# SAR-Research-Lab/lvt

Hardware: AMD Instinct MI355X
Metric: stereo frames/sec (KITTI-shaped 1241x376), per-frame SE3 vs CPU ref (higher is better)
Workload: dtype u8/f64

## Files before the change

include/lvt_amd_ext.h:

```cpp
#ifndef LVT_AMD_EXT_H__
#define LVT_AMD_EXT_H__

#include "lvt_c.h"
#include <stdint.h>

#ifdef __cplusplus
extern "C" {
#endif

typedef struct lvt_amd_params {
    float fx, fy, cx, cy;
    float baseline;
    int img_width, img_height;
    float k1, k2, p1, p2, k3;
    float near_plane_distance, far_plane_distance;
    float triangulation_ratio_test_threshold;
    float tracking_ratio_test_threshold;
    float descriptor_matching_threshold;
    int min_num_matches_for_tracking;
    int tracking_radius;
    int detection_cell_size;
    int max_keypoints_per_cell;
    int agast_threshold;
    int untracked_threshold;
    int staged_threshold;
    int triangulation_policy;
} lvt_amd_params;

LVT_API void lvt_amd_default_params(lvt_amd_params *p);
LVT_API int lvt_amd_params_from_file(const char *config_file_name, lvt_amd_params *p);
LVT_API lvt_handle lvt_amd_create(const lvt_amd_params *p, int sensor_type);
LVT_API lvt_handle lvt_amd_create_on_device(const lvt_amd_params *p, int sensor_type, int device);
LVT_API int lvt_amd_get_device(lvt_handle h);
LVT_API lvt_handle lvt_amd_create_pooled(const lvt_amd_params *p, int sensor_type, int device );
LVT_API void lvt_amd_reset(lvt_handle h);
LVT_API void lvt_amd_track_rgbd(lvt_handle h, const unsigned char *gray, const float *depth, int n_rows,
                                int n_cols, double R[3][3], double t[3]);
LVT_API void lvt_amd_track_device(lvt_handle h, const void *d_left, const void *d_right, int n_rows,
                                  int n_cols, int pitch_bytes, double R[3][3], double t[3]);
LVT_API void lvt_amd_track_device_async(lvt_handle h, const void *d_left, const void *d_right, int n_rows,
                                        int n_cols, int pitch_bytes);
LVT_API int lvt_amd_track_async(lvt_handle h, const unsigned char *left, const unsigned char *right, int n_rows, int n_cols);
LVT_API int lvt_amd_track_rgbd_async(lvt_handle h, const unsigned char *gray, const float *depth, int n_rows, int n_cols);
LVT_API void lvt_amd_wait(lvt_handle h, double R[3][3], double t[3]);
LVT_API int lvt_amd_wait_status(lvt_handle h, double R[3][3], double t[3]);
LVT_API int lvt_amd_wait_pose(lvt_handle h, double q_wxyz[4], double p[3]);
enum { LVT_AMD_DEPTH_F32 = 0, LVT_AMD_DEPTH_U16 = 1 };
LVT_API int lvt_amd_track_rgbd_device_async(lvt_handle h, const void *d_gray, int gray_pitch_bytes, const void *d_depth, int depth_pitch_bytes,
                                            int depth_format, float depth_scale, int n_rows, int n_cols);
LVT_API int lvt_amd_track_rgbd_device(lvt_handle h, const void *d_gray, int gray_pitch_bytes, const void *d_depth, int depth_pitch_bytes, int depth_format,
                                      float depth_scale, int n_rows, int n_cols, double R[3][3], double t[3]);
LVT_API int lvt_amd_track_rgbd16(lvt_handle h, const unsigned char *gray, const uint16_t *depth16, float depth_scale, int n_rows, int n_cols,
                                 double R[3][3], double t[3]);
LVT_API int lvt_amd_track_rgbd16_async(lvt_handle h, const unsigned char *gray, const uint16_t *depth16, float depth_scale, int n_rows, int n_cols);
LVT_API int lvt_amd_batch_track_rgbd_device_async(lvt_handle h, const void *const *d_gray, const void *const *d_depth, const int *n_rows, const int *n_cols,
                                                  const int *gray_pitch_bytes, const int *depth_pitch_bytes, int depth_format, float depth_scale);
LVT_API lvt_handle lvt_amd_batch_create(const lvt_amd_params *p, int sensor_type, int n_sequences);
LVT_API int lvt_amd_batch_size(lvt_handle h);
LVT_API void lvt_amd_batch_track_device_async(lvt_handle h, const void *const *d_left, const void *const *d_right,
                                              int n_rows, int n_cols, int pitch_bytes);
LVT_API void lvt_amd_batch_wait(lvt_handle h, double *R, double *t, int *status);
LVT_API void lvt_amd_batch_get_counts(lvt_handle h, int seq, int out[32]);
LVT_API lvt_handle lvt_amd_batch_create_mixed(const lvt_amd_params *p , int sensor_type, int n_sequences);
LVT_API int lvt_amd_batch_track_device_async_mixed(lvt_handle h, const void *const *d_left, const void *const *d_right,
                                                   const int *n_rows, const int *n_cols, const int *pitch_bytes);
LVT_API int lvt_amd_batch_get_params(lvt_handle h, int seq, lvt_amd_params *out);
LVT_API int lvt_amd_batch_mixed_tables(const lvt_amd_params *p, int sensor_type, int n_sequences, unsigned *cells, int cells_cap,
                                       unsigned *score, int score_cap, int counts[2]);

LVT_API void lvt_amd_set_stream(lvt_handle h, void *hip_stream);
LVT_API const char *lvt_amd_last_error(lvt_handle h);

LVT_API void lvt_amd_get_host_stats(lvt_handle h, long long out[8]);

LVT_API void lvt_amd_profile_enable(lvt_handle h, int enable);
LVT_API int lvt_amd_profile_read(lvt_handle h, int slot, char *name, int name_cap, double *total_ms, long *calls);

enum {
    LVT_AMD_C_N_LEFT = 0, LVT_AMD_C_N_RIGHT, LVT_AMD_C_MAP_SIZE, LVT_AMD_C_STAGED_SIZE, LVT_AMD_C_N_MATCHES,
    LVT_AMD_C_SECOND_PASS, LVT_AMD_C_N_ROW_MATCHES, LVT_AMD_C_N_TRIANGULATED, LVT_AMD_C_TRIANGULATED,
    LVT_AMD_C_RETRY_LEFT, LVT_AMD_C_RETRY_RIGHT, LVT_AMD_C_PNP_ITERS, LVT_AMD_C_PNP_INLIERS,
    LVT_AMD_C_MAP_SIZE_AT_MATCH, LVT_AMD_C_N_STAGED_ERASED, LVT_AMD_C_N_STAGED_PROMOTED, LVT_AMD_C_N_CULLED,
    LVT_AMD_C_FRAME, LVT_AMD_C_OVERFLOW ,
    LVT_AMD_C_PNP_BORDERLINE ,
    LVT_AMD_C_ROW_FALLBACK ,
    LVT_AMD_C_PNP_TRIALS , LVT_AMD_C_PNP_REJECTIONS ,
    LVT_AMD_C_PNP_TERMINATES ,
    LVT_AMD_C__COUNT = 32
};
LVT_API void lvt_amd_get_counts(lvt_handle h, int out[LVT_AMD_C__COUNT]);
LVT_API int lvt_amd_get_features(lvt_handle h, int eye, float *xy, float *resp, uint8_t *desc, int cap);
LVT_API int lvt_amd_get_matches(lvt_handle h, int *feat_idx, double *xyz, int cap);
LVT_API int lvt_amd_get_row_matches(lvt_handle h, int *pairs, int cap);
LVT_API int lvt_amd_get_map(lvt_handle h, double *xyz, int *counter, int *age, uint8_t *desc, int cap);
LVT_API int lvt_amd_get_staged(lvt_handle h, double *xyz, int *counter, uint8_t *desc, int cap);
LVT_API void lvt_amd_get_pose(lvt_handle h, double q_wxyz[4], double p[3]);
LVT_API int lvt_amd_get_last_pose(lvt_handle h, double q_wxyz[4], double p[3]);
LVT_API void lvt_amd_get_predicted_pose(lvt_handle h, double q_wxyz[4], double p[3]);
LVT_API void lvt_amd_get_debug(lvt_handle h, long long out[32]);
LVT_API void lvt_amd_get_timeline(lvt_handle h, long long out[16]);
LVT_API int lvt_amd_get_ordering(lvt_handle h);
LVT_API int lvt_amd_get_plane(lvt_handle h, int eye, int what, void *dst, int cap_bytes, int *pitch_out);

LVT_API int lvt_amd_pnp(const lvt_amd_params *p, const double q_in[4], const double p_in[3], const double *pts,
                        const float *obs, int n, double q_out[4], double p_out[3], int *n_solve_calls);
LVT_API int lvt_amd_pnp_detail(const lvt_amd_params *p, const double q_in[4], const double p_in[3], const double *pts,
                               const float *obs, int n, double q_out[4], double p_out[3], int *n_solve_calls,
                               double *err_out, int *level_out, int *borderline);
LVT_API int lvt_amd_pnp_trace(const lvt_amd_params *p, const double q_in[4], const double p_in[3], const double *pts,
                              const float *obs, int n, double q_out[4], double p_out[3], int *n_solve_calls,
                              double *err_out, int *level_out, int *borderline, double *trace, int trace_cap, int stats[3]);
LVT_API float lvt_amd_hamming_match_batched(const void *q_desc, const void *q_xy, const void *t_desc,
                                            const void *t_xy, const void *t_flag, int B, int M, int N,
                                            float r2, int mode, int img_rows, int img_cols, void *out,
                                            void *hip_stream);
LVT_API float lvt_amd_hamming_match_batched_n(const void *q_desc, const void *q_xy, const void *t_desc,
                                              const void *t_xy, const void *t_flag, int B, int M, int N,
                                              float r2, int mode, int img_rows, int img_cols, void *out,
                                              void *hip_stream, int launches);

typedef void *lvt_amd_rectifier;
LVT_API lvt_amd_rectifier lvt_amd_rectifier_create(const double K[9], const double D[5], const double R[9],
                                                   const double Pnew[9], int width, int height);
LVT_API void lvt_amd_rectifier_destroy(lvt_amd_rectifier r);
LVT_API int lvt_amd_rectify_device(lvt_amd_rectifier r, const void *d_src, int src_pitch, void *d_dst, int dst_pitch,
                                   void *hip_stream);
LVT_API int lvt_amd_rectify(lvt_amd_rectifier r, const unsigned char *src, unsigned char *dst);
LVT_API int lvt_amd_rectifier_get_maps(lvt_amd_rectifier r, float *map1, float *map2);

typedef void *lvt_amd_odometry;
LVT_API lvt_amd_odometry lvt_amd_odometry_create(lvt_handle h, const double base_to_sensor[12] , int reset_pose_on_lost);
LVT_API void lvt_amd_odometry_destroy(lvt_amd_odometry o);
LVT_API void lvt_amd_odometry_reset(lvt_amd_odometry o);
LVT_API int lvt_amd_odometry_push_pose(lvt_amd_odometry o, const double R[3][3], const double t[3], int status, double stamp_sec,
                                       double pose_out[7], double twist_out[6]);
LVT_API int lvt_amd_odometry_update(lvt_amd_odometry o, unsigned char *left, unsigned char *right, int n_rows, int n_cols, double stamp_sec,
                                    double pose_out[7], double twist_out[6]);

#ifdef __cplusplus
}
#endif
#endif
```

lvt_amd/__init__.py:

```python
from __future__ import annotations

import ctypes as C
import os

import numpy as np

from .params import LvtParameters, ParamsPOD, kitti_params, euroc_params, tum_params

_HERE = os.path.dirname(os.path.abspath(__file__))
LIB_PATH = os.environ.get("LVT_AMD_LIB") or os.path.join(_HERE, "lib", "liblvt_c.so")

ABI_SYMBOLS = [
    "lvt_create", "lvt_destroy", "lvt_track", "lvt_track_with_external_corners", "lvt_get_status",
    "lvt_amd_default_params", "lvt_amd_params_from_file", "lvt_amd_create", "lvt_amd_reset",
    "lvt_amd_track_rgbd", "lvt_amd_track_device", "lvt_amd_track_device_async", "lvt_amd_wait",
    "lvt_amd_set_stream", "lvt_amd_last_error", "lvt_amd_get_counts", "lvt_amd_get_features",
    "lvt_amd_get_matches", "lvt_amd_get_row_matches", "lvt_amd_get_map", "lvt_amd_get_staged",
    "lvt_amd_get_pose", "lvt_amd_get_last_pose", "lvt_amd_get_predicted_pose", "lvt_amd_get_plane", "lvt_amd_pnp", "lvt_amd_pnp_detail",
    "lvt_amd_hamming_match_batched", "lvt_amd_hamming_match_batched_n", "lvt_amd_rectifier_create", "lvt_amd_rectifier_destroy",
    "lvt_amd_rectify_device", "lvt_amd_rectify", "lvt_amd_rectifier_get_maps",
    "lvt_amd_odometry_create", "lvt_amd_odometry_destroy", "lvt_amd_odometry_reset", "lvt_amd_odometry_push_pose", "lvt_amd_odometry_update", "lvt_amd_profile_enable", "lvt_amd_profile_read", "lvt_amd_get_debug", "lvt_amd_get_timeline", "lvt_amd_get_ordering",
    "lvt_amd_batch_create", "lvt_amd_batch_size", "lvt_amd_batch_track_device_async", "lvt_amd_batch_wait",
    "lvt_amd_batch_get_counts", "lvt_amd_create_on_device", "lvt_amd_get_device", "lvt_amd_wait_status", "lvt_amd_get_host_stats",
    "lvt_amd_track_async", "lvt_amd_track_rgbd_async", "lvt_amd_pnp_trace", "lvt_amd_create_pooled", "lvt_amd_wait_pose",
    "lvt_amd_batch_create_mixed", "lvt_amd_batch_track_device_async_mixed", "lvt_amd_batch_get_params", "lvt_amd_batch_mixed_tables",
    "lvt_amd_track_rgbd_device", "lvt_amd_track_rgbd_device_async", "lvt_amd_track_rgbd16", "lvt_amd_track_rgbd16_async",
    "lvt_amd_batch_track_rgbd_device_async",
]

N_COUNTS = 32
COUNT_NAMES = ["n_left", "n_right", "map_size", "staged_size", "n_matches", "second_pass", "n_row_matches",
               "n_triangulated", "triangulated", "retry_left", "retry_right", "pnp_iters", "pnp_inliers",
               "map_size_at_match", "n_staged_erased", "n_staged_promoted", "n_culled", "frame", "overflow", "pnp_borderline", "row_fallback", "pnp_trials", "pnp_rejections", "pnp_terminates"]

eState_NOT_INITIALIZED, eState_TRACKING, eState_LOST = 1, 2, 3
eSensor_STEREO, eSensor_RGBD = 1, 2
DEPTH_F32, DEPTH_U16 = 0, 1

_lib = None


def load_library():
    global _lib
    if _lib is not None:
        return _lib
    if not os.path.exists(LIB_PATH):
        raise RuntimeError(f"{LIB_PATH} is missing: build it with `make -C lvt_amd/csrc` "
                           "(there is no CPU fallback for the tracking path)")
    try:
        import torch
    except Exception:
        pass
    L = C.CDLL(LIB_PATH)
    vp = C.c_void_p
    L.lvt_create.restype = vp
    L.lvt_create.argtypes = [C.c_char_p, C.c_int]
    L.lvt_amd_create.restype = vp
    L.lvt_amd_create.argtypes = [vp, C.c_int]
    L.lvt_amd_create_on_device.restype = vp
    L.lvt_amd_create_on_device.argtypes = [vp, C.c_int, C.c_int]
    L.lvt_amd_get_device.argtypes = [vp]
    L.lvt_amd_create_pooled.restype = vp
    L.lvt_amd_create_pooled.argtypes = [vp, C.c_int, C.c_int]
    L.lvt_destroy.argtypes = [vp]
    L.lvt_amd_reset.argtypes = [vp]
    L.lvt_track.argtypes = [vp, vp, vp, C.c_int, C.c_int, vp, vp]
    L.lvt_track_with_external_corners.argtypes = [vp, vp, vp, C.c_int, C.c_int, vp, C.c_int, vp, C.c_int, vp, vp]
    L.lvt_get_status.argtypes = [vp]
    L.lvt_amd_params_from_file.argtypes = [C.c_char_p, vp]
    L.lvt_amd_default_params.argtypes = [vp]
    L.lvt_amd_track_rgbd.argtypes = [vp, vp, vp, C.c_int, C.c_int, vp, vp]
    L.lvt_amd_track_device.argtypes = [vp, vp, vp, C.c_int, C.c_int, C.c_int, vp, vp]
    L.lvt_amd_track_device_async.argtypes = [vp, vp, vp, C.c_int, C.c_int, C.c_int]
    L.lvt_amd_wait.argtypes = [vp, vp, vp]
    L.lvt_amd_track_async.argtypes = [vp, vp, vp, C.c_int, C.c_int]
    L.lvt_amd_track_async.restype = C.c_int
    L.lvt_amd_track_rgbd_async.argtypes = [vp, vp, vp, C.c_int, C.c_int]
    L.lvt_amd_track_rgbd_async.restype = C.c_int
    L.lvt_amd_wait_status.argtypes = [vp, vp, vp]
    L.lvt_amd_wait_status.restype = C.c_int
    L.lvt_amd_set_stream.argtypes = [vp, vp]
    L.lvt_amd_last_error.restype = C.c_char_p
    L.lvt_amd_last_error.argtypes = [vp]
    L.lvt_amd_get_counts.argtypes = [vp, vp]
    L.lvt_amd_get_features.argtypes = [vp, C.c_int, vp, vp, vp, C.c_int]
    L.lvt_amd_get_matches.argtypes = [vp, vp, vp, C.c_int]
    L.lvt_amd_get_row_matches.argtypes = [vp, vp, C.c_int]
    L.lvt_amd_get_map.argtypes = [vp, vp, vp, vp, vp, C.c_int]
    L.lvt_amd_get_staged.argtypes = [vp, vp, vp, vp, C.c_int]
    L.lvt_amd_get_pose.argtypes = [vp, vp, vp]
    L.lvt_amd_get_last_pose.argtypes = [vp, vp, vp]
    L.lvt_amd_get_predicted_pose.argtypes = [vp, vp, vp]
    L.lvt_amd_get_plane.argtypes = [vp, C.c_int, C.c_int, vp, C.c_int, vp]
    L.lvt_amd_pnp.argtypes = [vp, vp, vp, vp, vp, C.c_int, vp, vp, vp]
    L.lvt_amd_pnp_detail.argtypes = [vp, vp, vp, vp, vp, C.c_int, vp, vp, vp, vp, vp, vp]
    L.lvt_amd_pnp_trace.argtypes = [vp, vp, vp, vp, vp, C.c_int, vp, vp, vp, vp, vp, vp, vp, C.c_int, vp]
    L.lvt_amd_hamming_match_batched.restype = C.c_float
    L.lvt_amd_hamming_match_batched.argtypes = [vp, vp, vp, vp, vp, C.c_int, C.c_int, C.c_int, C.c_float, C.c_int, C.c_int, C.c_int, vp, vp]
    L.lvt_amd_get_timeline.argtypes = [vp, vp]
    L.lvt_amd_get_ordering.argtypes = [vp]
    L.lvt_amd_get_ordering.restype = C.c_int
    L.lvt_amd_rectifier_create.restype = vp
    L.lvt_amd_rectifier_create.argtypes = [vp, vp, vp, vp, C.c_int, C.c_int]
    L.lvt_amd_rectifier_destroy.argtypes = [vp]
    L.lvt_amd_rectify_device.argtypes = [vp, vp, C.c_int, vp, C.c_int, vp]
    L.lvt_amd_rectify.argtypes = [vp, vp, vp]
    L.lvt_amd_rectifier_get_maps.argtypes = [vp, vp, vp]
    L.lvt_amd_odometry_create.restype = vp
    L.lvt_amd_odometry_create.argtypes = [vp, vp, C.c_int]
    L.lvt_amd_odometry_destroy.argtypes = [vp]
    L.lvt_amd_odometry_reset.argtypes = [vp]
    L.lvt_amd_odometry_push_pose.restype = C.c_int
    L.lvt_amd_odometry_push_pose.argtypes = [vp, vp, vp, C.c_int, C.c_double, vp, vp]
    L.lvt_amd_odometry_update.restype = C.c_int
    L.lvt_amd_odometry_update.argtypes = [vp, vp, vp, C.c_int, C.c_int, C.c_double, vp, vp]
    L.lvt_amd_hamming_match_batched_n.restype = C.c_float
    L.lvt_amd_hamming_match_batched_n.argtypes = [vp, vp, vp, vp, vp, C.c_int, C.c_int, C.c_int, C.c_float, C.c_int, C.c_int, C.c_int, vp, vp, C.c_int]
    L.lvt_amd_profile_enable.argtypes = [vp, C.c_int]
    L.lvt_amd_batch_create.restype = vp
    L.lvt_amd_batch_create.argtypes = [vp, C.c_int, C.c_int]
    L.lvt_amd_batch_size.argtypes = [vp]
    L.lvt_amd_batch_track_device_async.argtypes = [vp, vp, vp, C.c_int, C.c_int, C.c_int]
    L.lvt_amd_batch_wait.argtypes = [vp, vp, vp, vp]
    L.lvt_amd_batch_get_counts.argtypes = [vp, C.c_int, vp]
    L.lvt_amd_batch_create_mixed.restype = vp
    L.lvt_amd_batch_create_mixed.argtypes = [vp, C.c_int, C.c_int]
    L.lvt_amd_batch_track_device_async_mixed.restype = C.c_int
    L.lvt_amd_batch_track_device_async_mixed.argtypes = [vp, vp, vp, vp, vp, vp]
    L.lvt_amd_batch_get_params.restype = C.c_int
    L.lvt_amd_batch_get_params.argtypes = [vp, C.c_int, vp]
    L.lvt_amd_batch_mixed_tables.restype = C.c_int
    L.lvt_amd_batch_mixed_tables.argtypes = [vp, C.c_int, C.c_int, vp, C.c_int, vp, C.c_int, vp]
    L.lvt_amd_batch_size.restype = C.c_int
    for name, argtypes in (
            ("lvt_amd_track_rgbd_device_async", [vp, vp, C.c_int, vp, C.c_int, C.c_int, C.c_float, C.c_int, C.c_int]),
            ("lvt_amd_track_rgbd_device", [vp, vp, C.c_int, vp, C.c_int, C.c_int, C.c_float, C.c_int, C.c_int, vp, vp]),
            ("lvt_amd_track_rgbd16", [vp, vp, vp, C.c_float, C.c_int, C.c_int, vp, vp]),
            ("lvt_amd_track_rgbd16_async", [vp, vp, vp, C.c_float, C.c_int, C.c_int]),
            ("lvt_amd_batch_track_rgbd_device_async", [vp, vp, vp, vp, vp, vp, vp, C.c_int, C.c_float])):
        if hasattr(L, name):
            fn = getattr(L, name)
            fn.argtypes, fn.restype = argtypes, C.c_int
    L.lvt_amd_get_debug.argtypes = [vp, vp]
    L.lvt_amd_get_host_stats.argtypes = [vp, vp]
    L.lvt_amd_profile_read.argtypes = [vp, C.c_int, C.c_char_p, C.c_int, vp, vp]
    _lib = L
    return L


def _p(a):
    return a.ctypes.data_as(C.c_void_p) if a is not None else None


def _u8(img):
    a = np.ascontiguousarray(img, dtype=np.uint8)
    assert a.ndim == 2
    return a


class LvtSystem:

    def __init__(self, handle, sensor_type):
        self._h = handle
        self._sensor = sensor_type

    @classmethod
    def create(cls, params: LvtParameters, sensor_type: int = eSensor_STEREO, device: int = -1, pooled: bool = False) -> "LvtSystem":
        L = load_library()
        pod = params.to_pod()
        if pooled:
            h = L.lvt_amd_create_pooled(C.byref(pod), sensor_type, device)
        else:
            h = L.lvt_amd_create_on_device(C.byref(pod), sensor_type, device) if device >= 0 else L.lvt_amd_create(C.byref(pod), sensor_type)
        if not h:
            raise RuntimeError("lvt_amd_create failed (bad parameters, or no usable HIP device -- no CPU fallback)")
        return cls(h, sensor_type)

    @classmethod
    def create_from_file(cls, config_file: str, sensor_type: int = eSensor_STEREO) -> "LvtSystem":
        L = load_library()
        h = L.lvt_create(config_file.encode(), sensor_type)
        if not h:
            raise RuntimeError("lvt_create returned NULL")
        return cls(h, sensor_type)

    @staticmethod
    def destroy(system: "LvtSystem"):
        system.close()

    def close(self):
        if self._h:
            load_library().lvt_destroy(self._h)
            self._h = None

    def __del__(self):
        try:
            self.close()
        except Exception:
            pass

    def reset(self):
        load_library().lvt_amd_reset(self._h)

    def get_sensor_type(self):
        return self._sensor

    def device(self) -> int:
        return load_library().lvt_amd_get_device(self._h)

    def get_state(self):
        return load_library().lvt_get_status(self._h)

    def last_error(self) -> str:
        return load_library().lvt_amd_last_error(self._h).decode()

    def host_stats(self) -> dict:
        a = (C.c_longlong * 8)()
        load_library().lvt_amd_get_host_stats(self._h, a)
        return {"enqueued": int(a[0]), "collected": int(a[1]), "planes_in_place": int(a[2]), "planes_staged": int(a[3]),
                "async_host_frames": int(a[4]), "pulls_carried_by_the_previous_frame": int(a[5]), "score_pieces": int(a[6]), "event_ordering": int(a[7])}

    def track(self, img1, img2, depth_scale=None):
        R = np.zeros((3, 3)); t = np.zeros(3)
        a = _u8(img1)
        if self._sensor == eSensor_STEREO:
            b = _u8(img2)
            load_library().lvt_track(self._h, _p(a), _p(b), a.shape[0], a.shape[1], _p(R), _p(t))
        elif isinstance(img2, np.ndarray) and img2.dtype == np.uint16:
            if depth_scale is None:
                raise ValueError("a uint16 depth image needs depth_scale (metres per raw unit)")
            d = np.ascontiguousarray(img2)
            load_library().lvt_amd_track_rgbd16(self._h, _p(a), _p(d), float(depth_scale), a.shape[0], a.shape[1], _p(R), _p(t))
        else:
            d = np.ascontiguousarray(img2, dtype=np.float32)
            load_library().lvt_amd_track_rgbd(self._h, _p(a), _p(d), a.shape[0], a.shape[1], _p(R), _p(t))
        return R, t

    def track_with_external_corners(self, left, right, corners_left, corners_right):
        R = np.zeros((3, 3)); t = np.zeros(3)
        a, b = _u8(left), _u8(right)
        cl = np.ascontiguousarray(corners_left, dtype=np.float64).reshape(-1, 2)
        cr = np.ascontiguousarray(corners_right, dtype=np.float64).reshape(-1, 2)
        load_library().lvt_track_with_external_corners(self._h, _p(a), _p(b), a.shape[0], a.shape[1], _p(cl), len(cl),
                                                       _p(cr), len(cr), _p(R), _p(t))
        return R, t

    def track_device(self, d_left: int, d_right: int, rows: int, cols: int, pitch: int):
        R = np.zeros((3, 3)); t = np.zeros(3)
        load_library().lvt_amd_track_device(self._h, C.c_void_p(d_left), C.c_void_p(d_right), rows, cols, pitch, _p(R), _p(t))
        return R, t

    def track_device_async(self, d_left: int, d_right: int, rows: int, cols: int, pitch: int):
        load_library().lvt_amd_track_device_async(self._h, C.c_void_p(d_left), C.c_void_p(d_right), rows, cols, pitch)

    def track_rgbd_device(self, d_gray: int, d_depth: int, rows: int, cols: int, gray_pitch: int, depth_pitch: int, depth_format: int = DEPTH_F32,
                          depth_scale: float = 1.0):
        R = np.zeros((3, 3)); t = np.zeros(3)
        rc = load_library().lvt_amd_track_rgbd_device(self._h, C.c_void_p(d_gray), gray_pitch, C.c_void_p(d_depth), depth_pitch, depth_format,
                                                      float(depth_scale), rows, cols, _p(R), _p(t))
        return (R, t) if rc == 0 else None

    def track_rgbd_device_async(self, d_gray: int, d_depth: int, rows: int, cols: int, gray_pitch: int, depth_pitch: int, depth_format: int = DEPTH_F32,
                                depth_scale: float = 1.0) -> int:
        return load_library().lvt_amd_track_rgbd_device_async(self._h, C.c_void_p(d_gray), gray_pitch, C.c_void_p(d_depth), depth_pitch, depth_format,
                                                              float(depth_scale), rows, cols)

    def track_async(self, img1, img2, depth_scale=None) -> int:
        a = img1 if (isinstance(img1, np.ndarray) and img1.dtype == np.uint8 and img1.flags.c_contiguous) else _u8(img1)
        if self._sensor == eSensor_STEREO:
            b = img2 if (isinstance(img2, np.ndarray) and img2.dtype == np.uint8 and img2.flags.c_contiguous) else _u8(img2)
            return load_library().lvt_amd_track_async(self._h, _p(a), _p(b), a.shape[0], a.shape[1])
        if isinstance(img2, np.ndarray) and img2.dtype == np.uint16:
            if depth_scale is None:
                raise ValueError("a uint16 depth image needs depth_scale (metres per raw unit)")
            d = img2 if img2.flags.c_contiguous else np.ascontiguousarray(img2)
            return load_library().lvt_amd_track_rgbd16_async(self._h, _p(a), _p(d), float(depth_scale), a.shape[0], a.shape[1])
        d = img2 if (isinstance(img2, np.ndarray) and img2.dtype == np.float32 and img2.flags.c_contiguous) else np.ascontiguousarray(img2, dtype=np.float32)
        return load_library().lvt_amd_track_rgbd_async(self._h, _p(a), _p(d), a.shape[0], a.shape[1])

    def track_async_ptr(self, p_left: int, p_right: int, rows: int, cols: int) -> int:
        return load_library().lvt_amd_track_async(self._h, C.c_void_p(p_left), C.c_void_p(p_right), rows, cols)

    def wait(self):
        R = np.zeros((3, 3)); t = np.zeros(3)
        load_library().lvt_amd_wait(self._h, _p(R), _p(t))
        return R, t

    def wait_status(self):
        R = np.zeros((3, 3)); t = np.zeros(3)
        st = load_library().lvt_amd_wait_status(self._h, _p(R), _p(t))
        return R, t, st

    def set_stream(self, hip_stream: int):
        load_library().lvt_amd_set_stream(self._h, C.c_void_p(hip_stream))

    def counts(self):
        a = np.zeros(N_COUNTS, dtype=np.int32)
        load_library().lvt_amd_get_counts(self._h, _p(a))
        return {n: int(a[i]) for i, n in enumerate(COUNT_NAMES)}

    def features(self, eye=0, cap=16384):
        xy = np.zeros((cap, 2), np.float32); resp = np.zeros(cap, np.float32); desc = np.zeros((cap, 32), np.uint8)
        n = load_library().lvt_amd_get_features(self._h, eye, _p(xy), _p(resp), _p(desc), cap)
# ... 295 lines not shown
```

lvt_amd/csrc/k_features.hip:

```cpp
#include "lvt_dev.h"
#include "lvt_math.h"
#include <type_traits>

namespace lvt {

__constant__ signed char c_brief[256][4] = {
#include "../../include/lvt_brief256_pattern.inc"
};
constexpr signed char BRIEF_TABLE[256][4] = {
#include "../../include/lvt_brief256_pattern.inc"
};
constexpr int brief_max_offset() {
    int m = 0;
    for (int i = 0; i < 256; i++)
        for (int k = 0; k < 4; k++) m = (BRIEF_TABLE[i][k] > m) ? BRIEF_TABLE[i][k] : (-BRIEF_TABLE[i][k] > m) ? -BRIEF_TABLE[i][k] : m;
    return m;
}

constexpr int TS_W = 64, TS_H = 16, HALO = 4;
constexpr int TILE_W = TS_W + 2 * HALO;
constexpr int TILE_H = TS_H + 2 * HALO;

typedef short s16x2 __attribute__((ext_vector_type(2)));
__device__ __forceinline__ s16x2 pk_min(s16x2 a, s16x2 b) { return __builtin_elementwise_min(a, b); }
// ... 760 lines not shown
            const uint32_t a = abv[cur];
            const int rc = key_r(keys[cur]);
            if ((a & NONE) != NONE) {
                const int w = find_max((int)(a & NONE));
                if (rc < key_r(keys[w])) nms[cur] = (I)w;
                else nms[w] = (I)cur;
            }
            if (a & LEFT) {
                const uint32_t above_root = (uint32_t)nms[cur];
                const int t = find_max(cur - 1);
                if (above_root == MAXF) {
                    if (t != cur) {
                        if (rc < key_r(keys[t])) nms[cur] = (I)t;
                        else nms[t] = (I)cur;
                    }
                } else if (t != (int)above_root) {
                    if (key_r(keys[above_root]) < key_r(keys[t])) {
                        nms[above_root] = (I)t;
                        nms[cur] = (I)t;
                    } else {
                        nms[t] = (I)above_root;
                        nms[cur] = (I)above_root;
                    }
                }
            }
            if (cur == lastm) break;
            cur = (int)uf[cur];
        }
    }
    __syncthreads();

    STAMP(4);
    uint32_t *arr = uf;
    int n_kp = 0;
    for (int base = 0; base < n_raw; base += 1024) {
        const int i = base + tid;
        const bool keep = (i < n_raw) && ((uint32_t)nms[i] == MAXF);
        const uint32_t k = keep ? keys[i] : 0;
        int total;
        const int off = n_kp + block_excl_scan(keep ? 1 : 0, scan, &total);
        if (keep) arr[off] = k;
        n_kp += total;
    }
    __syncthreads();

    STAMP(5);
    return n_kp;
}

constexpr int ANMS_SORT = 1, ANMS_RADII = 2, ANMS_SELECT = 4, ANMS_ALL = 7;
template <typename I, int XB = 10>
__device__ __forceinline__ int cell_anms(const Seq &S, const CellGeom &g, uint32_t *keys, uint32_t *uf, I *root, I *abv, I *nms, int n_kp, int n_cap, int *row_first,
                                         int *row_end, int *scan, int *misc, float *out, long long *dbg, int n_raw_dbg, int parts = ANMS_ALL, int i_first = 0,
                                         int i_stride = 1) {
    constexpr uint32_t NONE = IdxT<I>::NONE, LEFT = IdxT<I>::LEFT, MAXF = IdxT<I>::MAXF;
    (void)NONE, (void)LEFT, (void)MAXF;
    const int tid = threadIdx.x;
    uint32_t *arr = uf;
    const int n_raw = n_raw_dbg;
    const int max_kp = S.prm.max_kp_cell;
    const float fX0 = (float)g.X0, fY0 = (float)g.Y0;
    int n_out = 0;
    if (n_kp > max_kp) {
        I *posL = root;
        I *posR = abv;
        uint32_t *sorted = keys;
        if (parts & ANMS_SORT) {
        {
            int *q = reinterpret_cast<int *>(nms);
            constexpr int DFS_AT = 64;
            constexpr int qcap = 2 * DFS_AT;
            static_assert((6 * qcap + 16 * 96) * sizeof(int) <= (size_t)RAW_CAP_SMALL * sizeof(uint16_t), "queues + stacks must fit the nms[] array of the smallest LDS instance");
            int *qa = q, *qb = q + 3 * qcap;
            int *stacks = q + 6 * qcap;
            const int nw = blockDim.x >> 6;
            if (tid == 0) {
                int depth0 = 0;
                for (int v = n_kp; v > 1; v >>= 1) depth0++;
                qa[0] = 0, qa[1] = n_kp, qa[2] = 2 * depth0;
                misc[1] = (n_kp > 16) ? 1 : 0;
                misc[2] = 0;
            }
            __syncthreads();
            int levels = 0;
            while (true) {
                const int cnt = misc[1];
                if (cnt == 0) break;
                levels++;
                if (cnt >= DFS_AT) {
                    for (int sgi = wave_id(); sgi < cnt; sgi += nw)
                        wave_introsort_segment<I>(arr, qa[3 * sgi], qa[3 * sgi + 1], qa[3 * sgi + 2], posL, posR, stacks + 96 * wave_id());
                    break;
                }
                for (int sgi = wave_id(); sgi < cnt; sgi += nw) {
                    const int first = qa[3 * sgi], last = qa[3 * sgi + 1], depth = qa[3 * sgi + 2];
                    if (depth == 0) {
                        if (lane_id() == 0) heap_sort_seq(arr + first, last - first);
                        continue;
                    }
                    const int cut = wave_partition_pivot<I>(arr, first, last, posL, posR);
                    if (lane_id() == 0) {
                        if (last - cut > 16) {
                            const int o = atomicAdd(&misc[2], 1);
                            qb[3 * o] = cut, qb[3 * o + 1] = last, qb[3 * o + 2] = depth - 1;
                        }
                        if (cut - first > 16) {
                            const int o = atomicAdd(&misc[2], 1);
                            qb[3 * o] = first, qb[3 * o + 1] = cut, qb[3 * o + 2] = depth - 1;
                        }
                    }
                }
                __syncthreads();
                if (tid == 0) {
                    misc[1] = misc[2];
                    misc[2] = 0;
                }
                int *t = qa;
                qa = qb;
                qb = t;
                __syncthreads();
            }
            __syncthreads();
            if (dbg && tid == 0) dbg[41] = levels;
        }
        STAMP(6);
        int *hist = row_first;
        int *gtab = row_end;
        const int nwv = blockDim.x >> 6;
        const bool par_rank = n_kp > 512 && (size_t)n_cap * sizeof(I) >= (size_t)nwv * 256 * sizeof(int);
        const int blk = par_rank ? (((n_kp + nwv - 1) / nwv + 63) & ~63) : n_kp;
        int *hw = par_rank ? reinterpret_cast<int *>(nms) : hist;
        if (par_rank) {
            for (int k = tid; k < nwv * 256; k += 1024) hw[k] = 0;
            __syncthreads();
        }
        if (par_rank || wave_id() == 0) {
            const int lane = lane_id();
            const uint64_t lt_mask = (lane == 0) ? 0ull : (~0ull >> (64 - lane));
            int *myh = par_rank ? hw + 256 * wave_id() : hist;
            if (!par_rank) {
                for (int k = lane; k < 256; k += 64) hist[k] = 0;
                __builtin_amdgcn_fence(__ATOMIC_ACQ_REL, "workgroup");
            }
            const int b_lo = par_rank ? wave_id() * blk : 0, b_hi = min(n_kp, b_lo + blk);
            for (int base = b_lo; base < b_hi; base += 64) {
                const int i = base + lane;
                const bool valid = i < b_hi;
                const int key = valid ? key_r(arr[i]) : 0;
                uint64_t m = __ballot(valid);
#pragma unroll
                for (int b = 0; b < 8; b++) {
                    const uint64_t bb = __ballot((key >> b) & 1);
                    m &= ((key >> b) & 1) ? bb : ~bb;
                }
                if (valid) {
                    const int hb = myh[key];
                    posL[i] = (I)(hb + __popcll(m & lt_mask));
                    if ((m & lt_mask) == 0ull) myh[key] = hb + __popcll(m);
                }
                __builtin_amdgcn_fence(__ATOMIC_ACQ_REL, "workgroup");
            }
        }
        if (par_rank) {
            __syncthreads();
            if (tid < 256) {
                int run = 0;
                for (int w = 0; w < nwv; w++) {
                    const int t = hw[256 * w + tid];
                    hw[256 * w + tid] = run;
                    run += t;
                }
                hist[tid] = run;
            }
            __syncthreads();
        }
        if (wave_id() == 0) {
            const int lane = lane_id();
            int h[4], tot = 0;
#pragma unroll
            for (int q = 0; q < 4; q++) {
                h[q] = hist[4 * lane + q];
                tot += h[q];
            }
            int incl = tot;
            for (int d = 1; d < 64; d <<= 1) {
                const int t = __shfl_down(incl, d, 64);
                if (lane + d < 64) incl += t;
            }
            int above = incl - tot;
#pragma unroll
            for (int q = 3; q >= 0; q--) {
                gtab[4 * lane + q] = above;
                above += h[q];
            }
        }
        __syncthreads();
        for (int i = tid; i < n_kp; i += 1024) {
            const uint32_t k = arr[i];
            const int kr = key_r(k);
            sorted[gtab[kr] + (par_rank ? hw[256 * (i / blk) + kr] : 0) + (int)posL[i]] = k;
        }
        __syncthreads();
        }
        STAMP(7);
        if (!(parts & (ANMS_RADII | ANMS_SELECT))) return n_kp;
        uint32_t *r2 = arr;
// ... 1036 lines not shown
```

lvt_amd/csrc/k_lists.hip:

```cpp
#include "lvt_dev.h"
#include "lvt_math.h"

namespace lvt {

constexpr int LS_THREADS = 512;
constexpr int LS_WAVES = LS_THREADS / 64;
constexpr int LS_TPT = 3;
constexpr int LS_NMAX = LS_THREADS * LS_TPT;
constexpr int LS_BINS = 1100;
constexpr int LS_QCH = 256;
constexpr int LS_SEG = 256;
constexpr int LS_STARTS = (LS_BINS + 4) & ~3;
constexpr int LS_LDS_BYTES = LS_NMAX * 42 + LS_STARTS * 4 + LS_QCH * 64 + LS_WAVES * LS_SEG * 4 + 256;
static_assert(KC + 64 <= LS_SEG, "the long-window path shares the wavefront's segment words");
typedef unsigned int ls_u32x4 __attribute__((ext_vector_type(4)));

__device__ __forceinline__ uint32_t ls_bcnt(uint32_t x, uint32_t acc) {
    uint32_t r;
    asm("v_bcnt_u32_b32 %0, %1, %2" : "=v"(r) : "v"(x), "v"(acc));
    return r;
}

template <int MODE, bool BV>
__global__ __launch_bounds__(LS_THREADS) void k_hamming_batched_lists(SeqArg<BV> sa, int par, seq_t seq) {
    const Seq &S = sa.get();
    Ctl &ctl = *S.ctl;
    const int tid = threadIdx.x, lane = tid & 63, wv = tid >> 6;
    int *fb = S.lists_fb + (MODE == MODE_ROW ? 1 : 0);
    int q_end = 0;
    if (MODE == MODE_MAP) {
        const int n_early = (ctl.gate_ok == seq) ? ctl.early_done : 0;
        if (n_early <= 0) return;
        q_end = min(*S.map_n, n_early);
    } else {
        if (S.prm.sensor != 1) return;
        if (seq && __hip_atomic_load(&S.fb[par].fc->feat_seq, __ATOMIC_ACQUIRE, __HIP_MEMORY_SCOPE_AGENT) < seq) return;
        q_end = *S.fb[par].feat[0].n;
    }
    const Feat &T = (MODE == MODE_ROW) ? S.fb[par].feat[1] : S.fb[par].feat[0];
    const int N = *T.n;
    const int ccx = S.prm.hash_ccx, ccy = S.prm.hash_ccy, csr = S.prm.cell_search_radius;
    const int nbins = (MODE == MODE_ROW) ? S.prm.H + 1 : ccx * ccy;
    if (N > LS_NMAX || nbins > LS_BINS || (MODE != MODE_ROW && csr > 2)) {
        if (tid == 0) *fb = 1;
        return;
    }
    if (tid == 0) *fb = 0;

    extern __shared__ __attribute__((aligned(16))) uint8_t smem[];
    ls_u32x4 *s_dlo = reinterpret_cast<ls_u32x4 *>(smem);
    ls_u32x4 *s_dhi = s_dlo + LS_NMAX;
    float2 *s_xy = reinterpret_cast<float2 *>(s_dhi + LS_NMAX);
    uint16_t *s_idx = reinterpret_cast<uint16_t *>(s_xy + LS_NMAX);
    int *s_start = reinterpret_cast<int *>(s_idx + LS_NMAX);
    ls_u32x4 *s_qd = reinterpret_cast<ls_u32x4 *>(s_start + LS_STARTS);
    ls_u32x4 *s_qw = s_qd + 2 * LS_QCH;
    uint32_t *s_seg = reinterpret_cast<uint32_t *>(s_qw + 2 * LS_QCH) + wv * LS_SEG;
    __shared__ int s_scan[32];
    __shared__ double w2c[12];

    long long *stamp = (MODE == MODE_ROW && blockIdx.x == 0 && tid == 0) ? ctl.dbg + 26 : nullptr;
    if (stamp) stamp[0] = clock64();
    float tx[LS_TPT], ty[LS_TPT];
    int tbin[LS_TPT], trank[LS_TPT];
    ls_u32x4 tlo[LS_TPT], thi[LS_TPT];
#pragma unroll
    for (int k = 0; k < LS_TPT; k++) {
        const int jc = max(min(tid + k * LS_THREADS, N - 1), 0);
        tx[k] = ty[k] = 0.f, tbin[k] = trank[k] = 0;
        tlo[k] = thi[k] = ls_u32x4{0, 0, 0, 0};
        if (N > 0) {
            tx[k] = T.x[jc], ty[k] = T.y[jc];
            if (MODE != MODE_ROW) tbin[k] = min(max((int)T.hcy[jc], 0), ccy - 1) * ccx + min(max((int)T.hcx[jc], 0), ccx - 1);
            const ls_u32x4 *d = reinterpret_cast<const ls_u32x4 *>(T.desc + (size_t)jc * 4);
            tlo[k] = d[0], thi[k] = d[1];
        }
    }
    if (MODE == MODE_MAP && tid == 0) {
        Pose predicted;
        double mmn[14];
        motion_predict(ctl, ctl.last_pose, predicted, mmn);
        world_to_camera(predicted, w2c);
    }
    for (int i = tid; i <= nbins; i += LS_THREADS) s_start[i] = 0;
    __syncthreads();
#pragma unroll
    for (int k = 0; k < LS_TPT; k++) {
        if (MODE == MODE_ROW) tbin[k] = min(max((int)floorf(ty[k]), 0), nbins - 1);
        if (tid + k * LS_THREADS < N) trank[k] = atomicAdd(&s_start[tbin[k]], 1);
    }
    __syncthreads();
    {
        const int chunk = (nbins + 1 + LS_THREADS - 1) / LS_THREADS;
        const int i0 = min(tid * chunk, nbins + 1), i1 = min(i0 + chunk, nbins + 1);
        int sum = 0;
        for (int i = i0; i < i1; i++) sum += s_start[i];
        int total;
        int run = block_excl_scan(sum, s_scan, &total);
        for (int i = i0; i < i1; i++) {
            const int v = s_start[i];
            s_start[i] = run;
            run += v;
        }
    }
    __syncthreads();
#pragma unroll
    for (int k = 0; k < LS_TPT; k++) {
        const int j = tid + k * LS_THREADS;
        if (j < N) {
            const int pos = s_start[tbin[k]] + trank[k];
            s_xy[pos] = make_float2(tx[k], ty[k]);
            s_idx[pos] = (uint16_t)j;
            s_dlo[pos] = tlo[k];
// ... 212 lines not shown
```

lvt_amd/csrc/k_track.hip:

```cpp
#include "lvt_dev.h"
#include "wave_reduce.h"
#include "lvt_math.h"

namespace lvt {

enum : int { MODE_MAP = 0, MODE_STAGED = 1, MODE_ROW = 2 };

__device__ __forceinline__ void frame_prologue(const Seq &S, Ctl &c, int par, const Pose &predicted, const double mm_next[14], bool active,
                                               bool first, bool skipped) {
    const bool absent = skipped && S.fb[par].fc->absent != 0;
    if (!absent) {
        for (int i = 0; i < N_COUNTS; i++) c.counts[i] = 0;
        c.counts[C_FRAME] = c.frame_number;
        c.frame_number++;
    }
    c.active = active ? 1 : 0;
    c.first_frame = first ? 1 : 0;
    c.do_pass2 = 0;
    c.n_pass1 = c.n_pass2 = 0;
    c.n_matches = 0;
    c.lost_now = 0;
    c.need_tri = 0;
    c.dont_stage = 0;
    c.n_pairs = 0;
// ... 345 lines not shown
            __threadfence();
            break;
        }
    }
}
__global__ __launch_bounds__(64) void k_gate_buf(Seq *seqs, seq_t want, int par) {
    if (threadIdx.x != 0) return;
    gate_buf_wait(seq_const(seqs, blockIdx.z), want, par);
}

__global__ void k_feat_done(Seq *seqs, int par, seq_t seq) {
    if (threadIdx.x != 0) return;
    FeatCtl &fc = *seq_const(seqs, blockIdx.x).fb[par].fc;
    seq_const(seqs, blockIdx.x).ctl->dbg[47] = (long long)wall_clock64();
    if (fc.poison) {
        fc.skip_seq = seq;
        fc.poison = 0;
    }
    __threadfence();
    atomicExch(&fc.feat_seq, seq);
}

__global__ void k_row_done(Seq *seqs, int par, seq_t seq) {
    if (threadIdx.x != 0) return;
    FeatCtl &fc = *seq_const(seqs, blockIdx.x).fb[par].fc;
    if (__hip_atomic_load(&fc.feat_seq, __ATOMIC_ACQUIRE, __HIP_MEMORY_SCOPE_AGENT) < seq) return;
    __threadfence();
    atomicExch(&fc.row_seq, seq);
}

template <bool BV>
__global__ __launch_bounds__(64) void k_gate(SeqArg<BV> sa, int par, seq_t want, seq_t seq, int test_timeout) {
    if (threadIdx.x == 0 && blockIdx.x == 0) sa.get().ctl->dbg[32] = (long long)wall_clock64();
    Ctl &ctl = *sa.get().ctl;
    FeatCtl &fc = *sa.get().fb[par].fc;
    if (threadIdx.x != 0) return;
    bool ok = true;
    if (test_timeout) {
        atomicAdd(&ctl.gate_timeouts, 1);
        ok = false;
    } else {
        const unsigned long long t0 = wall_clock64();
        while (__hip_atomic_load(&fc.feat_seq, __ATOMIC_ACQUIRE, __HIP_MEMORY_SCOPE_AGENT) < seq) {
            __builtin_amdgcn_s_sleep(8);
            if (wall_clock64() - t0 > 2000000ull) {
                atomicAdd(&ctl.gate_timeouts, 1);
                ok = false;
                break;
            }
        }
        if (ok && __hip_atomic_load(&fc.skip_seq, __ATOMIC_ACQUIRE, __HIP_MEMORY_SCOPE_AGENT) == seq) ok = false;
        const unsigned long long t1 = wall_clock64();
        ctl.dbg[35] = (long long)t1;
        while (ok && __hip_atomic_load(&ctl.pnp_seq, __ATOMIC_ACQUIRE, __HIP_MEMORY_SCOPE_AGENT) < want) {
            __builtin_amdgcn_s_sleep(8);
            if (wall_clock64() - t1 > 2000000ull) {
                atomicAdd(&ctl.gate_timeouts, 1);
                ok = false;
                break;
            }
        }
    }
    const seq_t mine = 4u * seq + (ok ? 1u : 3u);
    seq_t cur = __hip_atomic_load(&ctl.early_state, __ATOMIC_ACQUIRE, __HIP_MEMORY_SCOPE_AGENT);
    for (;;) {
        if (cur >= 4u * seq + 1u) {
            ok = false;
            break;
        }
        const seq_t seen = atomicCAS(&ctl.early_state, cur, mine);
        if (seen == cur) break;
        cur = seen;
    }
    ctl.gate_ok = ok ? seq : (seq_t)0;
    ctl.dbg[33] = (long long)wall_clock64();
}

template <bool BV>
__global__ __launch_bounds__(256) void k_early_map(SeqArg<BV> sa, int par, seq_t seq, int only_fb) {
    if (threadIdx.x == 0 && blockIdx.x == 0) sa.get().ctl->dbg[34] = (long long)wall_clock64();
    const Seq &S = sa.get();
    if (only_fb && !S.lists_fb[0]) return;
    Ctl &ctl = *S.ctl;
    const int n_early = (ctl.gate_ok == seq) ? ctl.early_done : 0;
    if (n_early <= 0) return;
    __shared__ double w2c[12];
    if (threadIdx.x == 0) {
        Pose predicted;
        double mmn[14];
        motion_predict(ctl, ctl.last_pose, predicted, mmn);
        world_to_camera(predicted, w2c);
    }
    __shared__ uint32_t lbuf[4 * KC];
    __shared__ float s_tx[NF_MAX], s_ty[NF_MAX];
    __shared__ uint32_t s_tc[NF_MAX];
    CandLds C;
    C.lbuf = lbuf, C.tx = s_tx, C.ty = s_ty, C.tc = s_tc, C.w2c = w2c;
    candidates_body<MODE_MAP, true>(S, 0, par, C, blockIdx.x * 4 + wave_id(), gridDim.x * 4, 256, 0, n_early);
}

template <int MODE>
__device__ void wave_top2_slow(const Query &q, const Feat &T, int N, const uint8_t *flag_lds, uint32_t &k1, uint32_t &k2, int &cnt) {
    const int lane = lane_id();
    uint32_t b1 = 0xFFFFFFFFu, b2 = 0xFFFFFFFFu;
    int c = 0;
    for (int base = 0; base < N; base += 64) {
        const int j = base + lane;
        if (j < N && !flag_lds[j] && cand_pred<MODE>(q, T, j)) {
            uint64_t t[4];
#pragma unroll
            for (int k = 0; k < 4; k++) t[k] = T.desc[(size_t)j * 4 + k];
            const uint32_t key = ((uint32_t)hamming256(q.d, t) << 16) | (uint32_t)j;
            if (key < b1) {
                b2 = b1;
                b1 = key;
            } else if (key < b2)
                b2 = key;
            c++;
        }
    }
    for (int d = 32; d >= 1; d >>= 1) {
        const uint32_t o1 = __shfl_xor(b1, d, 64), o2 = __shfl_xor(b2, d, 64);
        const int oc = __shfl_xor(c, d, 64);
        const uint32_t n1 = min(b1, o1);
        const uint32_t n2 = min(max(b1, o1), min(b2, o2));
        b1 = n1;
        b2 = n2;
        c += oc;
    }
    k1 = b1;
    k2 = b2;
    cnt = c;
}

__device__ __forceinline__ bool accept_match(int cnt, uint32_t k1, uint32_t k2, float ratio_th, float desc_th) {
    if (cnt > 1) {
        const float d1 = (float)(k1 >> 16), d2 = (float)(k2 >> 16);
        return (d1 / d2) < ratio_th;
    }
    if (cnt == 1) return (float)(k1 >> 16) <= desc_th;
    return false;
}

__device__ __forceinline__ void wave_first_two(uint32_t c0, uint32_t c1, bool v0, bool v1, uint32_t &k1, uint32_t &k2, int &cnt) {
    const uint64_t m0 = __ballot(v0), m1 = __ballot(v1);
    cnt = __popcll(m0) + __popcll(m1);
    int s1 = -1, s2 = -1;
    uint64_t a = m0, b = m1;
    if (a) {
        s1 = __ffsll((long long)a) - 1;
        a &= a - 1;
    } else if (b) {
        s1 = 64 + __ffsll((long long)b) - 1;
        b &= b - 1;
    }
    if (a) s2 = __ffsll((long long)a) - 1;
    else if (b) s2 = 64 + __ffsll((long long)b) - 1;
    k1 = k2 = 0xFFFFFFFFu;
    if (s1 >= 0) k1 = (s1 < 64) ? __shfl(c0, s1, 64) : __shfl(c1, s1 - 64, 64);
    if (s2 >= 0) k2 = (s2 < 64) ? __shfl(c0, s2, 64) : __shfl(c1, s2 - 64, 64);
}

constexpr int RES_THREADS = 1024;
constexpr int QCAP = 2 * RES_THREADS;
constexpr int LCAP = 24576;

struct ResolveLds {
    uint8_t *flag;
    uint32_t *tab0;
    uint32_t *tab1;
    uint32_t *lists;
    int *scan;
    int *misc;
};

template <int MODE>
__device__ __forceinline__ int decide_query_slow(const Seq &S, const Feat &T, int N, const uint8_t *flag, const uint64_t *qdesc, int i,
                                                 float qx, float qy, int radius, float ratio, float desc_th) {
    Query q;
    if (MODE == MODE_ROW) make_query_row(S.prm, qx, qy, q);
    else make_query_track(S.prm, qx, qy, radius, q);
#pragma unroll
    for (int k = 0; k < 4; k++) q.d[k] = qdesc[(size_t)i * 4 + k];
    uint32_t k1, k2;
    int cnt;
    wave_top2_slow<MODE>(q, T, N, flag, k1, k2, cnt);
    return accept_match(cnt, k1, k2, ratio, desc_th) ? (int)(k1 & 0xFFFFu) : -1;
}

constexpr uint32_t PERM = 0xFFFFFFFFu;

template <class NFn>
__device__ __forceinline__ int resolve_super(int b0, int M, NFn nfn, const uint32_t *cand, ResolveLds &L, uint32_t &iter, float ratio,
                                             float desc_th, int acc[2], int nq[2] = nullptr, const uint32_t *qidx = nullptr, int qid[2] = nullptr,
                                             bool no_marks = false) {
    const int tid = threadIdx.x;
    int n[2], off[2], qq[2];
    const long long ts0 = clock64();
    if (tid == 0) L.misc[0] = QCAP;
    __syncthreads();
#pragma unroll
    for (int u = 0; u < 2; u++) {
        const int lq = tid + u * RES_THREADS, q = b0 + lq;
        qq[u] = q;
        if (qidx) {
            const uint32_t w = (q < M) ? qidx[q] : 0u;
            qq[u] = (int)(w & 0xFFFFFFu);
            n[u] = (int)(w >> 24);
        } else
            n[u] = (q < M) ? nfn(q) : 0;
        if (n[u] > KC) atomicMin(&L.misc[0], lq);
    }
    if (qid) qid[0] = qq[0], qid[1] = qq[1];
    __syncthreads();
    int limit = min(min(QCAP, M - b0), L.misc[0]);
    if (limit == 0) return -1;
#pragma unroll
    for (int u = 0; u < 2; u++)
        if (tid + u * RES_THREADS >= limit) n[u] = 0;
    const int n4[2] = {(n[0] + 3) & ~3, (n[1] + 3) & ~3};
    int t0, t1;
    off[0] = block_excl_scan(n4[0], L.scan, &t0);
    if (limit > RES_THREADS) {
        off[1] = t0 + block_excl_scan(n4[1], L.scan, &t1);
    } else {
        off[1] = t0;
        t1 = 0;
    }
    if (t0 + t1 > LCAP) {
        int f0 = (tid < limit && off[0] + n4[0] <= LCAP) ? 1 : 0, f1 = (tid + RES_THREADS < limit && off[1] + n4[1] <= LCAP) ? 1 : 0;
        int c0, c1;
        block_excl_scan(f0, L.scan, &c0);
        block_excl_scan(f1, L.scan, &c1);
        limit = (c0 < min(limit, RES_THREADS)) ? c0 : c0 + c1;
#pragma unroll
        for (int u = 0; u < 2; u++)
            if (tid + u * RES_THREADS >= limit) n[u] = 0;
    }
    const long long ts1 = clock64();
    if (nq) nq[0] = n[0], nq[1] = n[1];
#pragma unroll
    for (int u = 0; u < 2; u++) {
        const uint4 *src = reinterpret_cast<const uint4 *>(cand + (size_t)qq[u] * KC);
        uint32_t *dst = L.lists + off[u];
        int w = 0;
        for (int e0 = 0; e0 < n[u]; e0 += 32) {
            uint4 v[8];
#pragma unroll
            for (int k = 0; k < 8; k++) v[k] = (e0 + 4 * k < n[u]) ? src[(e0 >> 2) + k] : make_uint4(0, 0, 0, 0);
            if (no_marks) {
#pragma unroll
                for (int k = 0; k < 8; k++)
                    if (e0 + 4 * k < n[u]) *reinterpret_cast<uint4 *>(dst + e0 + 4 * k) = v[k];
                w = n[u];
                continue;
            }
            uint32_t mk[32];
#pragma unroll
            for (int k = 0; k < 8; k++) {
                if (e0 + 4 * k < n[u]) {
                    mk[4 * k] = L.tab0[v[k].x & (uint32_t)(NF_MAX - 1)];
                    mk[4 * k + 1] = L.tab0[v[k].y & (uint32_t)(NF_MAX - 1)];
                    mk[4 * k + 2] = L.tab0[v[k].z & (uint32_t)(NF_MAX - 1)];
                    mk[4 * k + 3] = L.tab0[v[k].w & (uint32_t)(NF_MAX - 1)];
                }
            }
#pragma unroll
            for (int k = 0; k < 8; k++) {
                const int e = e0 + 4 * k;
                if (e < n[u]) {
                    if (mk[4 * k] != PERM) dst[w++] = v[k].x;
                    if (e + 1 < n[u] && mk[4 * k + 1] != PERM) dst[w++] = v[k].y;
                    if (e + 2 < n[u] && mk[4 * k + 2] != PERM) dst[w++] = v[k].z;
                    if (e + 3 < n[u] && mk[4 * k + 3] != PERM) dst[w++] = v[k].w;
                }
            }
        }
        n[u] = w;
    }
    if (tid == 0) L.misc[12] = L.misc[13] = QCAP;
    __syncthreads();
    int prev[2] = {-2, -2};
    acc[0] = acc[1] = -1;
    int dbg_steps = 0;
    const long long tj0 = clock64();
    const uint32_t it0 = iter;
    int fin = 0;
    while (true) {
        iter++;
        const uint32_t *rd = (iter & 1u) ? L.tab0 : L.tab1;
        uint32_t *wr = (iter & 1u) ? L.tab1 : L.tab0;
        int first_changed = QCAP;
#pragma unroll
        for (int u = 0; u < 2; u++) {
            const int lq = tid + u * RES_THREADS;
            if (n[u] == 0 || lq < fin) continue;
            const uint32_t *list = L.lists + off[u];
            const uint32_t mine = ((iter - 1u) << 11) | (uint32_t)(2047 - lq);
            uint32_t k1 = 0xFFFFFFFFu, k2 = 0xFFFFFFFFu;
            int cnt = 0;
            for (int e = 0; e < n[u] && cnt < 2; e += 4) {
                uint32_t c[4], v[4];
                {
                    const uint4 c4 = *reinterpret_cast<const uint4 *>(list + e);
                    c[0] = c4.x, c[1] = c4.y, c[2] = c4.z, c[3] = c4.w;
                }
#pragma unroll
                for (int k = 0; k < 4; k++) v[k] = rd[c[k] & (uint32_t)(NF_MAX - 1)];
#pragma unroll
                for (int k = 0; k < 4; k++) {
                    const bool un = v[k] > mine;
                    if (e + k < n[u] && !un && cnt < 2) {
                        if (cnt == 0) k1 = c[k];
                        else k2 = c[k];
                        cnt++;
                    }
                }
            }
            const bool ok = accept_match(cnt, k1, k2, ratio, desc_th);
            dbg_steps = max(dbg_steps, n[u]);
            acc[u] = ok ? (int)(k1 & 0xFFFFu) : -1;
            if (ok) atomicMax(&wr[acc[u]], (iter << 11) | (uint32_t)(2047 - lq));
            if (acc[u] != prev[u]) first_changed = min(first_changed, lq);
            prev[u] = acc[u];
        }
        int *slot = &L.misc[12 + (iter & 1u)];
        if (first_changed < QCAP) atomicMin(slot, first_changed);
        __syncthreads();
        const int fc = *slot;
        if (fc >= QCAP) break;
        if (tid == 0) L.misc[12 + ((iter + 1u) & 1u)] = QCAP;
#pragma unroll
        for (int u = 0; u < 2; u++) {
            const int lq = tid + u * RES_THREADS;
            if (lq >= fin && lq < fc && n[u] > 0 && acc[u] >= 0) {
                L.flag[acc[u]] = 1;
                L.tab0[acc[u]] = PERM;
                L.tab1[acc[u]] = PERM;
            }
        }
        fin = fc;
        __syncthreads();
    }
    if (threadIdx.x == 0) {
        L.misc[4] = (int)(iter - it0);
        L.misc[5] = (int)(clock64() - tj0);
        L.misc[6] = (int)(ts1 - ts0);
        L.misc[3] = 0;
        L.misc[7] = (int)(tj0 - ts1);
    }
    __syncthreads();
    {
        int m = dbg_steps;
        for (int d = 32; d >= 1; d >>= 1) m = max(m, __shfl_xor(m, d, 64));
        if (lane_id() == 0) atomicMax(&L.misc[3], m);
    }
#pragma unroll
    for (int u = 0; u < 2; u++)
        if (acc[u] >= 0) {
            L.flag[acc[u]] = 1;
            L.tab0[acc[u]] = PERM;
// ... 303 lines not shown
        int m = S.match[i], cnt = A.counter[i], ag = A.age[i];
        if (m == -1) cnt += 1;
        else if (m >= 0) ag += 1;
        if (lost) {
            A.match_idx[i] = m, A.counter[i] = cnt, A.age[i] = ag;
            continue;
        }
        if (!mt && !kp) continue;
        const double p0 = A.pos[3 * i], p1 = A.pos[3 * i + 1], p2 = A.pos[3 * i + 2];
        if (mt && offm < NF_MAX) {
            S.pnp_X[3 * offm] = p0;
            S.pnp_X[3 * offm + 1] = p1;
            S.pnp_X[3 * offm + 2] = p2;
            S.pnp_obs[2 * offm] = F.x[m];
            S.pnp_obs[2 * offm + 1] = F.y[m];
            S.pnp_feat[offm] = m;
            S.pnp_level[offm] = 0;
        }
        if (kp) {
            B.pos[3 * offk] = p0, B.pos[3 * offk + 1] = p1, B.pos[3 * offk + 2] = p2;
#pragma unroll
            for (int q = 0; q < 4; q++) B.desc[(size_t)offk * 4 + q] = A.desc[(size_t)i * 4 + q];
            B.counter[offk] = cnt;
            B.age[offk] = ag;
            B.match_idx[offk] = m;
        } else if (mt)
            S.fb[par].feat[0].flag[m] = 0;
    }
    if (lost) return true;
    __syncthreads();
    if (tid == 0) {
        ctl.counts[C_N_CULLED] = M - n_keep;
        *S.map_cur = cur ^ 1;
        *S.map_n = n_keep;
    }
    return false;
}

template <bool BV>
__global__ __launch_bounds__(RES_THREADS) void k_track_mid(SeqArg<BV> sa, int par, seq_t seq) {
    if (threadIdx.x == 0 && blockIdx.x == 0) sa.get().ctl->dbg[42] = (long long)wall_clock64();
    const Seq &S = sa.get();
    Ctl &ctl = *S.ctl;
    if (!ctl.active) return;
    if (threadIdx.x == 0 && ctl.mm_pending) {
        for (int k = 0; k < 4; k++) ctl.mm_last_q[k] = ctl.mm_next[k], ctl.mm_ang_vel[k] = ctl.mm_next[4 + k];
        for (int k = 0; k < 3; k++) ctl.mm_last_p[k] = ctl.mm_next[8 + k], ctl.mm_lin_vel[k] = ctl.mm_next[11 + k];
        ctl.mm_pending = 0;
    }
    if (ctl.first_frame) return;
    RESOLVE_LDS_DECL
    {
        const int n_early = (ctl.early_ran_seq == seq) ? max(ctl.early_done, 0) : 0;
        resolve_body<MODE_MAP>(S, ctl, 0, par, L, r_tab, n_early > 0 ? 2 : 0, n_early);
        __syncthreads();
        if (threadIdx.x == 0) ctl.early_done = 0;
    }
    __syncthreads();
    if (L.misc[2]) {
        {
            CandLds C;
            C.lbuf = r_lists;
            C.tx = reinterpret_cast<float *>(r_lists + 16 * KC);
            C.ty = C.tx + NF_MAX;
            C.tc = reinterpret_cast<uint32_t *>(C.ty + NF_MAX);
            candidates_body<MODE_MAP>(S, 1, par, C, wave_id(), RES_THREADS / 64, RES_THREADS);
        }
        __syncthreads();
        resolve_body<MODE_MAP>(S, ctl, 1, par, L, r_tab);
        __syncthreads();
    }
    if (*S.map_n <= RES_THREADS) {
        bookkeep_cull_small(S, ctl, par, L.scan);
        return;
    }
    bookkeep_cull_large(S, ctl, par, L.scan, L.lists);
}

template <bool BV>
__global__ __launch_bounds__(RES_THREADS) void k_early_mid(SeqArg<BV> sa, int par, seq_t seq) {
    if (threadIdx.x == 0 && blockIdx.x == 0) sa.get().ctl->dbg[36] = (long long)wall_clock64();
    const Seq &S = sa.get();
    Ctl &ctl = *S.ctl;
    const int n_early = (ctl.gate_ok == seq) ? ctl.early_done : 0;
    if (n_early > 0) {
        RESOLVE_LDS_DECL
        resolve_body<MODE_MAP>(S, ctl, 0, par, L, r_tab, 1, n_early);
        __syncthreads();
        if (threadIdx.x == 0) ctl.early_ran_seq = seq;
    }
    if (threadIdx.x == 0) {
        ctl.dbg[37] = (long long)wall_clock64();
        __threadfence();
        if (n_early > 0 || ctl.gate_ok == seq) atomicCAS(&ctl.early_state, 4u * seq + 1u, 4u * seq + 2u);
    }
}

__device__ __forceinline__ void deliver_record(const Ctl &ctl, Ctl *rec_out, seq_t *done_out, seq_t seq, int nthreads) {
    static_assert(sizeof(Ctl) % 8 == 0, "record copy");
    const unsigned long long *src = reinterpret_cast<const unsigned long long *>(&ctl);
    unsigned long long *dst = reinterpret_cast<unsigned long long *>(rec_out);
    for (int i = threadIdx.x; i < (int)(sizeof(Ctl) / 8); i += nthreads) dst[i] = __hip_atomic_load(&src[i], __ATOMIC_RELAXED, __HIP_MEMORY_SCOPE_AGENT);
    __threadfence_system();
    __syncthreads();
    if (threadIdx.x == 0) __hip_atomic_store(done_out, seq, __ATOMIC_RELEASE, __HIP_MEMORY_SCOPE_SYSTEM);
}
__global__ __launch_bounds__(64) void k_deliver(Seq *seqs, Ctl *rec_out, seq_t *done_out, seq_t seq) {
    deliver_record(*seq_const(seqs, blockIdx.z).ctl, rec_out + blockIdx.z, done_out + blockIdx.z, seq, 64);
}

__device__ __forceinline__ void gate_late_poll(Ctl &ctl, FeatCtl &fc, seq_t seq) {
    unsigned long long t0 = wall_clock64();
    for (;;) {
        const seq_t cur = __hip_atomic_load(&ctl.early_state, __ATOMIC_ACQUIRE, __HIP_MEMORY_SCOPE_AGENT);
        if (cur >= 4u * seq + 2u) break;
        __builtin_amdgcn_s_sleep(8);
        if (wall_clock64() - t0 > 6000000ull) {
            atomicAdd(&ctl.gate_timeouts, 1);
            if (cur < 4u * seq + 1u && atomicCAS(&ctl.early_state, cur, 4u * seq + 3u) == cur) break;
            t0 = wall_clock64();
        }
    }
    t0 = wall_clock64();
    while (__hip_atomic_load(&fc.feat_seq, __ATOMIC_ACQUIRE, __HIP_MEMORY_SCOPE_AGENT) < seq) {
        __builtin_amdgcn_s_sleep(8);
        if (wall_clock64() - t0 > 200000000ull) {
            ctl.skip = 1;
            atomicAdd(&ctl.gate_fatal, 1);
            break;
        }
    }
    if (__hip_atomic_load(&fc.skip_seq, __ATOMIC_ACQUIRE, __HIP_MEMORY_SCOPE_AGENT) == seq) ctl.skip = 1;
}

template <bool BV>
__global__ __launch_bounds__(64) void k_gate_late(SeqArg<BV> sa, int par, seq_t seq, Ctl *prev_rec, seq_t *prev_done) {
    if (threadIdx.x == 0 && blockIdx.x == 0) sa.get().ctl->dbg[38] = (long long)wall_clock64();
    Ctl &ctl = *sa.get().ctl;
    FeatCtl &fc = *sa.get().fb[par].fc;
    if (prev_rec) deliver_record(ctl, prev_rec + blockIdx.z, prev_done + blockIdx.z, seq - 1, 64);
    if (threadIdx.x == 0) gate_late_poll(ctl, fc, seq);
}

__device__ __forceinline__ double rcp_nr(double s) {
    double y = __builtin_amdgcn_rcp(s);
#pragma unroll
    for (int it = 0; it < 2; it++) y = __builtin_fma(__builtin_fma(-s, y, 1.0), y, y);
    return y;
}
__device__ __forceinline__ double log_ge1(double a) {
    int e = __builtin_amdgcn_frexp_exp(a);
    double m = __builtin_amdgcn_frexp_mant(a);
    const bool lo = m < 0.70710678118654752440;
    m = lo ? m + m : m;
    e = lo ? e - 1 : e;
    const double s = (m - 1.0) * rcp_nr(m + 1.0);
    const double z = s * s;
    double p = 1.0 / 21.0;
    p = __builtin_fma(p, z, 1.0 / 19.0);
    p = __builtin_fma(p, z, 1.0 / 17.0);
    p = __builtin_fma(p, z, 1.0 / 15.0);
    p = __builtin_fma(p, z, 1.0 / 13.0);
    p = __builtin_fma(p, z, 1.0 / 11.0);
    p = __builtin_fma(p, z, 1.0 / 9.0);
    p = __builtin_fma(p, z, 1.0 / 7.0);
    p = __builtin_fma(p, z, 1.0 / 5.0);
    p = __builtin_fma(p, z, 1.0 / 3.0);
    const double sz = s * z;
    const double ed = (double)e;
    return __builtin_fma(ed, 6.93147180369123816490e-01, (s + s) + __builtin_fma(ed, 1.90821492927058770002e-10, (sz + sz) * p));
}
__device__ __forceinline__ double rsqrt_nr(double s) {
    double y = __builtin_amdgcn_rsq(s);
#pragma unroll
    for (int it = 0; it < 2; it++) {
        const double e = __builtin_fma(-(s * y), y, 1.0);
        y = __builtin_fma(0.5 * y, e, y);
// ... 350 lines not shown
                ok = sh.ok != 0;
                have_sys = speculate && (sh.accepted != 0);
                __syncthreads();
            } while (cont);
        }
        {
            int kept = 0;
            for (int i = tid; i < n; i += PNP_THREADS) {
                if (level[i] != 0) continue;
                const double e0 = err[2 * i], e1 = err[2 * i + 1];
                const double e2 = e0 * e0 + e1 * e1;
                bool out = e2 > REPROJ_TH2;
                if (fabs(e2 - REPROJ_TH2) < PNP_GATE_MARGIN) {
                    const double *gw = sh.cam[sw_slot];
                    double wi[12];
                    for (int j = 0; j < 4; j++) {
                        wi[j] = fx * gw[j] + cx * gw[8 + j];
                        wi[4 + j] = fy * gw[4 + j] + cy * gw[8 + j];
                        wi[8 + j] = gw[8 + j];
                    }
                    const double x = X[3 * i], y = X[3 * i + 1], z = X[3 * i + 2];
                    const double px = ((wi[0] * x + wi[1] * y) + wi[2] * z) + wi[3];
                    const double py = ((wi[4] * x + wi[5] * y) + wi[6] * z) + wi[7];
                    const double pz = ((wi[8] * x + wi[9] * y) + wi[10] * z) + wi[11];
                    const double r0 = px / pz - (double)obs[2 * i], r1 = py / pz - (double)obs[2 * i + 1];
                    out = (r0 * r0 + r1 * r1) > REPROJ_TH2;
                    n_border[0] += 1.0;
                }
                if (out) level[i] = 1;
                else kept = 1;
            }
            any_active = __syncthreads_or(kept) != 0;
        }
    }
    {
        double cnt[1] = {65536.0 * n_border[0]};
        for (int i = tid; i < n; i += PNP_THREADS) cnt[0] += (level[i] == 0) ? 1.0 : 0.0;
        block_sum<1>(cnt, red);
        const long long packed = (long long)cnt[0];
        inliers = (int)(packed & 65535), borderline = (int)(packed >> 16);
    }
    solve_calls = calls;
    for (int k = 0; k < 4; k++) result.q[k] = sh.r[k];
    for (int k = 0; k < 3; k++) result.p[k] = sh.t[k];
    if (dbg && tid == 0) {
        dbg[12] = t_sweep, dbg[13] = t_red, dbg[14] = t_solve, dbg[15] = t_dec, dbg[16] = clock64() - t_all, dbg[17] = calls;
    }
    __syncthreads();
}

constexpr int PNP_STAGE_MAX = 1536;
constexpr int PNP_DYN_BYTES = PNP_STAGE_MAX * (24 + 16 + 8 + 1);

__device__ __forceinline__ void pnp_solve(const Params &prm, const Pose &prior, const double *X, const float *obs, double *err, int8_t *level,
                                          int n, PnpShared &sh, double *red, uint8_t *dyn, Pose &res, int &inliers, int &calls, int &borderline, long long *dbg, bool copy_out) {
    if (n <= PNP_STAGE_MAX) {
        double *sX = reinterpret_cast<double *>(dyn);
        double *sErr = sX + 3 * PNP_STAGE_MAX;
        float *sObs = reinterpret_cast<float *>(sErr + 2 * PNP_STAGE_MAX);
        int8_t *sLvl = reinterpret_cast<int8_t *>(sObs + 2 * PNP_STAGE_MAX);
        for (int i = threadIdx.x; i < 3 * n; i += PNP_THREADS) sX[i] = X[i];
        for (int i = threadIdx.x; i < 2 * n; i += PNP_THREADS) sObs[i] = obs[i];
        for (int i = threadIdx.x; i < n; i += PNP_THREADS) sLvl[i] = level[i];
        __syncthreads();
        pnp_run(prm, prior, sX, sObs, sErr, red + PNP_RED - 2, sLvl, n, sh, red, res, inliers, calls, borderline, dbg);
        if (copy_out) {
            for (int i = threadIdx.x; i < 2 * n; i += PNP_THREADS) err[i] = sErr[i];
            for (int i = threadIdx.x; i < n; i += PNP_THREADS) level[i] = sLvl[i];
        }
    } else
        pnp_run(prm, prior, X, obs, err, err + 2 * (size_t)n, level, n, sh, red, res, inliers, calls, borderline, dbg);
}

struct PoseRec {
    double R[9], t[3];
    double q[4], p[3];
    int status, pad;
};
template <bool BV>
__global__ __launch_bounds__(PNP_THREADS) void k_pnp(SeqArg<BV> sa, int par, seq_t seq, PoseRec *pose_out, seq_t *pose_done) {
    if (threadIdx.x == 0 && blockIdx.x == 0) sa.get().ctl->dbg[44] = (long long)wall_clock64();
    const Seq &S = sa.get();
    Ctl &ctl = *S.ctl;
    if (!ctl.active || ctl.first_frame || ctl.lost_now) {
        if (threadIdx.x == 0) {
            __threadfence();
            atomicExch(&ctl.pnp_seq, seq);
        }
        return;
    }
    __shared__ PnpShared sh;
    __shared__ double red[PNP_RED];
    extern __shared__ __attribute__((aligned(16))) uint8_t pnp_dyn[];
    Pose res;
    int inliers, calls, borderline;
    if (threadIdx.x == 0) sh.trace = nullptr, sh.trace_cap = 0;
    pnp_solve(S.prm, ctl.predicted, S.pnp_X, S.pnp_obs, S.pnp_err, S.pnp_level, ctl.n_matches, sh, red, pnp_dyn, res, inliers, calls, borderline, ctl.dbg, false);
    if (threadIdx.x == 0) {
        ctl.optimized = res;
        ctl.last_pose = res;
        pose_to_Rt(res, ctl.out_R, ctl.out_t);
        ctl.out_status = 2;
        ctl.counts[C_PNP_ITERS] = calls;
        ctl.counts[C_PNP_INLIERS] = inliers;
        ctl.counts[C_PNP_BORDERLINE] = borderline;
        ctl.counts[C_PNP_TRIALS] = sh.trials, ctl.counts[C_PNP_REJECTIONS] = sh.rejections, ctl.counts[C_PNP_TERMINATES] = sh.terminates;
        ctl.early_done = *S.map_n;
        ctl.early_accepted = 0;
        ctl.dbg[45] = (long long)wall_clock64();
        __threadfence();
        atomicExch(&ctl.pnp_seq, seq);
        if (pose_out) {
            PoseRec &o = pose_out[blockIdx.z];
            for (int k = 0; k < 9; k++) o.R[k] = ctl.out_R[k];
            for (int k = 0; k < 3; k++) o.t[k] = ctl.out_t[k];
            for (int k = 0; k < 4; k++) o.q[k] = res.q[k];
            for (int k = 0; k < 3; k++) o.p[k] = res.p[k];
            o.status = 2;
            __threadfence_system();
            __hip_atomic_store(&pose_done[blockIdx.z], seq, __ATOMIC_RELEASE, __HIP_MEMORY_SCOPE_SYSTEM);
        }
    }
    if (S.prm.staged_th > 0) project_staged(S, res, red);
}

__global__ __launch_bounds__(PNP_THREADS) void k_pnp_standalone(Params prm, Pose prior, const double *X, const float *obs, double *err,
                                                                int8_t *level, int n, Pose *out, int *info, double *trace, int trace_cap) {
    __shared__ PnpShared sh;
    __shared__ double red[PNP_RED];
    extern __shared__ __attribute__((aligned(16))) uint8_t pnp_dyn[];
    for (int i = threadIdx.x; i < n; i += PNP_THREADS) level[i] = 0;
    if (threadIdx.x == 0) sh.trace = trace, sh.trace_cap = trace_cap;
    __syncthreads();
    Pose res;
    int inliers, calls, borderline;
    pnp_solve(prm, prior, X, obs, err, level, n, sh, red, pnp_dyn, res, inliers, calls, borderline, nullptr, true);
    if (threadIdx.x == 0) {
        *out = res;
        info[0] = calls;
        info[1] = inliers;
        info[2] = borderline;
        info[3] = sh.trials, info[4] = sh.rejections, info[5] = sh.terminates;
    }
}

__device__ __forceinline__ void staged_body(const Seq &S, Ctl &ctl, int par, ResolveLds &L, uint32_t *r_tab) {
    const int tid = threadIdx.x;
    if (!ctl.first_frame && S.prm.staged_th > 0) {
        const Feat &T = S.fb[par].feat[0];
        const int N = *T.n;
        const int scur = *S.staged_cur, SM = *S.staged_n;
        const MapSoA &A = S.staged[scur], &B = S.staged[scur ^ 1];
        const MapSoA &MP = S.map[*S.map_cur];
        if (SM > 0) {
        for (int j = tid; j < NF_MAX; j += RES_THREADS) {
            const uint8_t f = (j < N) ? T.flag[j] : 0;
            if (j < N) L.flag[j] = f;
            r_tab[j] = r_tab[NF_MAX + j] = f ? PERM : 0u;
        }
        const int map_n0 = *S.map_n;
        uint32_t iter = 0;
        int matched_before = 0, promoted_before = 0, erased = 0;
        bool map_ovf = false;
        __syncthreads();
        for (int b0 = 0; b0 < SM;) {
            int acc[2];
// ... 340 lines not shown
```

lvt_amd/csrc/lvt_dev.h:

```cpp
#pragma once
#include <hip/hip_runtime.h>
#include <stdint.h>

namespace lvt {

constexpr int NF_MAX = 4096;
constexpr int CELLS_MAX = 64;
constexpr int CELL_OUT_CAP = 2048;
constexpr int RAW_CAP = 10240;
constexpr int CELL_SIDE_LDS = 1024;
constexpr int CELL_SIDE_MAX = 4096;
constexpr int MAP_MAX = 32768;
constexpr int STAGED_MAX = 16384;
constexpr int KC = 128;
constexpr int N_COUNTS = 32;

enum : int { OVF_RAW = 1, OVF_CELL_OUT = 2, OVF_FEATURES = 4, OVF_MAP = 8, OVF_STAGED = 16, OVF_CELL_DIM = 32 };

enum : int {
    C_N_LEFT = 0, C_N_RIGHT, C_MAP_SIZE, C_STAGED_SIZE, C_N_MATCHES, C_SECOND_PASS, C_N_ROW_MATCHES,
    C_N_TRIANGULATED, C_TRIANGULATED, C_RETRY_LEFT, C_RETRY_RIGHT, C_PNP_ITERS, C_PNP_INLIERS,
    C_MAP_SIZE_AT_MATCH, C_N_STAGED_ERASED, C_N_STAGED_PROMOTED, C_N_CULLED, C_FRAME, C_OVERFLOW, C_PNP_BORDERLINE,
    C_ROW_FALLBACK,
    C_PNP_TRIALS, C_PNP_REJECTIONS, C_PNP_TERMINATES
};

constexpr double REPROJ_TH2 = 5.991;
constexpr double PNP_GATE_MARGIN = 1e-8;
constexpr int N_MAP_POINTS = 250;
constexpr int ROW_RADIUS = 2;
constexpr int HASH_CELL = 25;
constexpr int CORNERS_LOW_TH = 200;
constexpr int N_MATCHES_TH = 50;

struct Params {
    float fx, fy, cx, cy, baseline;
    float k1, k2, p1, p2, k3;
    float near_plane, far_plane;
    float tri_ratio, track_ratio, desc_th;
    float min_x, max_x, min_y, max_y;
    int W, H;
    int min_matches, tracking_radius, cell_size, max_kp_cell, agast_th, agast_th_low;
    int untracked_th, staged_th, tri_policy;
    int cells_x, cells_y, n_cells;
    int hash_ccx, hash_ccy, cell_search_radius;
    int sensor;
    int undistort;
    unsigned cell_magic;
    int big_cell_strips;
};

struct Pose {
    double q[4];
    double p[3];
};

using seq_t = unsigned long long;

struct Ctl {
    int state;
    int frame_number;
    int last_matches[3];
    Pose last_pose;
    double mm_last_q[4], mm_ang_vel[4], mm_last_p[3], mm_lin_vel[3];
    double mm_next[14];
    int mm_pending;
    int early_done;
    int early_accepted;
    seq_t pnp_seq, gate_ok, early_ran_seq;
    seq_t early_state;
    seq_t track_done_seq;
    seq_t late_gate_seq;
    int gate_timeouts;
    int gate_fatal;
    int skip;
    int active;
    int first_frame;
    int do_pass2;
    int n_pass1, n_pass2;
    int n_matches;
    int lost_now;
    int need_tri;
    int dont_stage;
    int n_pairs;
    Pose predicted, optimized;
    int counts[N_COUNTS];
    int overflow;
    long long dbg[48];
    double out_R[9], out_t[3];
    int out_status;
};

constexpr int NPAR = 3;

struct FeatCtl {
    int ext_corners;
    int n_ext[2];
    int n_detected[2];
    int retry[2];
    int overflow;
    seq_t row_seq;
    unsigned done_blocks;
    int absent;
    int poison;
    seq_t skip_seq;
    seq_t feat_seq;
};

enum { DEPTH_F32 = 0, DEPTH_U16 = 1 };

struct Feat {
    float *x, *y, *resp;
    float *bx, *by;
    float *depth;
    uint64_t *desc;
    uint8_t *flag;
    int16_t *hcx, *hcy;
    int *n;
};

struct MapSoA {
    double *pos;
    uint64_t *desc;
    int *counter, *age, *match_idx;
};

struct FrameBuf {
    const uint8_t *img[2];
    const float *depth_img;
    int img_pitch, depth_pitch;
    int depth_format;
    float depth_scale;
    uint8_t *score[2];
    uint16_t *boxsum[2];
    uint32_t *seg_keys[2];
    uint16_t *seg_cnt[2];
    float *cell_kp[2];
    int *cell_n[2];
    const float *ext_xy[2];
    const float *ext_xy_own[2];
    Feat feat[2];
    FeatCtl *fc;
};

struct Seq {
    Params prm;
    Ctl *ctl;
    FrameBuf fb[NPAR];
    int plane_pitch;
    uint32_t *cell_scratch[2];
    size_t cell_scratch_off[CELLS_MAX];
    uint32_t *strip_kp[2];
    int *strip_n[2];
    int *cell_big[2];
    int *lists_fb;
// ... 71 lines not shown
```

lvt_amd/csrc/lvt_host.hip:

```cpp
#define LVT_EXPORT_FUNCTIONS
#include "../../include/lvt_amd_ext.h"

#include "k_features.hip"
#include "k_track.hip"
#include "k_hamming.hip"
#include "k_lists.hip"
#include "k_rectify.hip"
#include "lvt_odometry.h"

#include <atomic>
#include <cmath>
#include <chrono>
#include <cstdio>
#include <cstdlib>
#include <cstring>
#include <string>
#include <functional>
#include <vector>

namespace lvt {

#define HIPCHK(ctx, call)                                                                  \
    do {                                                                                   \
        hipError_t e__ = (call);                                                           \
// ... 17 lines not shown
}
constexpr int FEAT_PACK = 32;
struct FrameArgsPack {
    FrameArgs a[FEAT_PACK];
};
static_assert(sizeof(Seq *) + sizeof(FrameArgsPack) + sizeof(int) + 2 * sizeof(seq_t) < 4096, "k_feat_begin_pack's arguments must stay under 4096 bytes");
__global__ void k_feat_begin_pack(Seq *seqs, FrameArgsPack pk, int par, seq_t want) {
    if (threadIdx.x != 0) return;
    if (want) gate_buf_wait(seq_const(seqs, blockIdx.x), want, par);
    const FrameArgs f = pk.a[blockIdx.x];
    feat_begin(seqs[blockIdx.x], f, par);
}

__global__ __launch_bounds__(256) void k_stage_in(const uint8_t *src0, const uint8_t *src1, uint8_t *dst0, uint8_t *dst1, int W, int H, int pitch) {
    stage_in_body(blockIdx.y ? src1 : src0, blockIdx.y ? dst1 : dst0, W, H, pitch, (size_t)blockIdx.x * blockDim.x + threadIdx.x, (size_t)gridDim.x * blockDim.x);
}
template <typename T>
__global__ __launch_bounds__(256) void k_stage_copy(const T *src, T *dst, size_t n) {
    constexpr size_t PER = 16 / sizeof(T);
    union Vec {
        uint4 q;
        T e[PER];
    };
    const size_t head = min((size_t)(((16 - ((uintptr_t)src & 15)) & 15) / sizeof(T)), n);
    const size_t nv = (n - head) / PER, tail0 = head + nv * PER;
    const size_t t0 = (size_t)blockIdx.x * blockDim.x + threadIdx.x, stride = (size_t)gridDim.x * blockDim.x;
    for (size_t v = t0; v < nv; v += stride) {
        Vec u;
        u.q = *reinterpret_cast<const uint4 *>(src + head + v * PER);
        T *d = dst + head + v * PER;
#pragma unroll
        for (size_t k = 0; k < PER; k++) d[k] = u.e[k];
    }
    if (t0 < head) dst[t0] = src[t0];
    if (t0 < n - tail0) dst[tail0 + t0] = src[tail0 + t0];
}
static void launch_stage_copy(hipStream_t st, const uint8_t *src, float *d_dst, size_t n, int fmt) {
    if (fmt == DEPTH_U16) hipLaunchKernelGGL(k_stage_copy<uint16_t>, dim3(256), dim3(256), 0, st, reinterpret_cast<const uint16_t *>(src), reinterpret_cast<uint16_t *>(d_dst), n);
    else hipLaunchKernelGGL(k_stage_copy<float>, dim3(256), dim3(256), 0, st, reinterpret_cast<const float *>(src), d_dst, n);
}

constexpr int MAX_DEVICES = 64;
static std::atomic<int> g_live_contexts[MAX_DEVICES];

constexpr uint64_t CTX_MAGIC = 0x4C56545F43545831ull, SLOT_MAGIC = 0x4C56545F534C5431ull;

struct Context {
    uint64_t magic = CTX_MAGIC;
    double host_enq_us = 0, host_wait_us = 0;
    long host_enq_n = 0, host_wait_n = 0;
    int gate_timeouts_seen = 0, gate_fatal_seen = 0;
    bool want_events = false, ordering_forced = false;
    hipEvent_t ev_switch = nullptr, ev_switch_e = nullptr;
    long test_gate_timeout = 0, switched_at = -1;
    long long planes_in_place = 0, planes_staged = 0;
    int device = 0;
    int B = 1;
    int launch_seqs = 0;
    int ring_seqs[8] = {};
    int sensor = 1;
    Params prm{};
    bool mixed = false;
    std::vector<Params> prms;
    std::vector<lvt_amd_params> in_prms;
    uint32_t *d_score_tab = nullptr, *d_cells_tab = nullptr;
    int n_score_wgs = 0, n_cells_wgs = 0;
    bool any_staged = false, any_strips = false;
    int max_cells = 0;
    const Params &seq_prm(int s) const { return mixed ? prms[s] : prm; }
    hipStream_t stream = nullptr;
    hipStream_t stream_f = nullptr;
    hipStream_t stream_e = nullptr;
    bool own_stream = false;
    std::vector<void *> allocs;
    Seq *d_seqs = nullptr;
    std::vector<Seq> h_seqs;
    std::vector<Ctl *> d_ctl;
    Ctl *h_ctl = nullptr;
    Ctl *h_ctl_dev = nullptr;
    seq_t *h_done = nullptr, *h_done_dev = nullptr;
    PoseRec *h_pose = nullptr, *h_pose_dev = nullptr;
    seq_t *h_pose_done = nullptr, *h_pose_done_dev = nullptr;
    bool binned_lists = false;
    bool early_pose = true;
    bool early_pending = false;
    FrameArgs *h_fargs = nullptr;
    hipEvent_t ev_done[RING] = {};
    bool events_only = false;
    CellOrder cell_order;
    int brief_from_image = 0;
    int score_pieces = 1;
    bool score_pieces_auto = true;
    double gate_balance_us = 0;
    int cells_raw_cap = RAW_CAP;
    unsigned cell_token = 0;
    int cell_split = 2;
    int lists_wgs_row = LISTS_WGS_ROW, lists_wgs_map = LISTS_WGS_MAP;
    int match_blocks_batch = 32;
    bool force_row_fallback = false;
    hipEvent_t ev_feat[NPAR] = {};
    hipEvent_t ev_depth = nullptr;
    bool depth_wait = false;
    std::function<void()> before_gather;
    uint8_t *d_img[NPAR][2] = {};
    uint8_t *h_stage[NPAR] = {}, *h_stage_dev[NPAR] = {};
    size_t stage_img = 0;
    float *d_depth[NPAR] = {};
    uint8_t *d_img_ring[RING][2] = {};
    float *d_depth_ring[RING] = {};
    uint8_t *h_stage_ring[RING] = {}, *h_stage_ring_dev[RING] = {};
    size_t stage_ring_bytes = 0;
    long long async_frames = 0;
    struct PendingFrame {
        bool valid = false, pulled = false;
        FrameArgs f{};
        const uint8_t *src[2] = {nullptr, nullptr};
        uint8_t *dst[2] = {nullptr, nullptr};
    } pend;
    NextPull next_pull{};
    bool fuse_pull = true;
    long long fused_pulls = 0;
    int feature_cus = 0;
    float *d_ext[NPAR][2] = {};
    int pitch = 0;
    long enq = 0, done = 0;
    long delivered = 0;
    bool sync_call = false;
    int last_slot = 0, last_par = 0;
    std::string err;
    bool prof = false;
    static constexpr int PROF_SLOTS = 24;
    hipEvent_t ev[PROF_SLOTS][2] = {};
    bool ev_used[PROF_SLOTS] = {};
    double prof_ms[PROF_SLOTS] = {};
    long prof_calls[PROF_SLOTS] = {};

    void set_error(const std::string &s) { err = s; }

    template <typename T>
    T *dalloc_uncached(size_t n) {
        void *p = nullptr;
        size_t bytes = ((n * sizeof(T) + 255) / 256) * 256;
        if (bytes == 0) bytes = 256;
        HIPCHK(this, hipExtMallocWithFlags(&p, bytes, hipDeviceMallocUncached));
        HIPCHK(this, hipMemset(p, 0, bytes));
        allocs.push_back(p);
        return static_cast<T *>(p);
    }
    template <typename T>
    T *dalloc(size_t n) {
        void *p = nullptr;
        size_t bytes = ((n * sizeof(T) + 255) / 256) * 256;
        if (bytes == 0) bytes = 256;
        HIPCHK(this, hipMalloc(&p, bytes));
        HIPCHK(this, hipMemset(p, 0, bytes));
        allocs.push_back(p);
        return static_cast<T *>(p);
    }

    bool counted = false;
    void count_in(int dev) {
        device = dev;
        g_live_contexts[dev % MAX_DEVICES].fetch_add(1);
        counted = true;
    }
    int live_on_device() const { return g_live_contexts[device % MAX_DEVICES].load(); }
// ... 105 lines not shown
}

static bool params_from_file(const char *fname, lvt_amd_params *p) {
    FILE *f = fname ? std::fopen(fname, "r") : nullptr;
    if (!f) return false;
    std::vector<std::pair<std::string, double>> kv;
    char line[1024];
    while (std::fgets(line, sizeof(line), f)) {
        char *hash = std::strchr(line, '#');
        if (hash) *hash = 0;
        char *colon = std::strchr(line, ':');
        if (!colon || line[0] == '%') continue;
        std::string key(line, colon - line);
        size_t a = key.find_first_not_of(" \t"), b = key.find_last_not_of(" \t");
        if (a == std::string::npos) continue;
        key = key.substr(a, b - a + 1);
        char *end = nullptr;
        double v = std::strtod(colon + 1, &end);
        if (end == colon + 1) continue;
        kv.emplace_back(key, v);
    }
    std::fclose(f);
    auto get = [&](const char *k) -> double {
        for (auto &e : kv)
            if (e.first == k) return e.second;
        return 0.0;
    };
    auto geti = [&](const char *k) -> int { return (int)std::nearbyint(get(k)); };
    p->fx = (float)get("fx"), p->fy = (float)get("fy"), p->cx = (float)get("cx"), p->cy = (float)get("cy");
    p->k1 = (float)get("k1"), p->k2 = (float)get("k2"), p->p1 = (float)get("p1"), p->p2 = (float)get("p2"), p->k3 = (float)get("k3");
    p->baseline = (float)get("baseline");
    p->img_width = geti("img_width"), p->img_height = geti("img_height");
    p->near_plane_distance = (float)get("near_plane_distance");
    p->far_plane_distance = (float)get("far_plane_distance");
    p->triangulation_ratio_test_threshold = (float)get("triangulation_ratio_test_threshold");
    p->tracking_ratio_test_threshold = (float)get("tracking_ratio_test_threshold");
    p->min_num_matches_for_tracking = geti("min_num_matches_for_tracking");
    p->tracking_radius = geti("tracking_radius");
    p->agast_threshold = geti("agast_threshold");
    p->untracked_threshold = geti("untracked_threshold");
    p->staged_threshold = geti("staged_threshold");
    p->descriptor_matching_threshold = (float)get("descriptor_matching_threshold");
    p->detection_cell_size = geti("detection_cell_size");
    p->max_keypoints_per_cell = geti("max_keypoints_per_cell");
    p->triangulation_policy = geti("triangulation_policy");
    return true;
}

static void alloc_feat(Context *c, Feat &F) {
    F.x = c->dalloc<float>(NF_MAX), F.y = c->dalloc<float>(NF_MAX), F.resp = c->dalloc<float>(NF_MAX);
    F.bx = c->dalloc<float>(NF_MAX), F.by = c->dalloc<float>(NF_MAX), F.depth = c->dalloc<float>(NF_MAX);
    F.desc = c->dalloc<uint64_t>((size_t)NF_MAX * 4);
    F.flag = c->dalloc<uint8_t>(NF_MAX);
    F.hcx = c->dalloc<int16_t>(NF_MAX), F.hcy = c->dalloc<int16_t>(NF_MAX);
    F.n = c->dalloc<int>(1);
}
static void alloc_points(Context *c, MapSoA &P, int cap) {
    P.pos = c->dalloc<double>((size_t)cap * 3);
    P.desc = c->dalloc<uint64_t>((size_t)cap * 4);
    P.counter = c->dalloc<int>(cap), P.age = c->dalloc<int>(cap), P.match_idx = c->dalloc<int>(cap);
}

static void drain(Context *c);

static void reset_state(Context *c, int only = -1) {
    drain(c);
    if (only < 0) c->gate_timeouts_seen = 0, c->gate_fatal_seen = 0;
    for (int s = 0; s < c->B; s++) {
        if (only >= 0 && s != only) continue;
        Ctl z;
        std::memset(&z, 0, sizeof(z));
        z.state = 1;
        z.last_matches[0] = z.last_matches[1] = z.last_matches[2] = 0x7FFFFFFF;
        z.last_pose.q[0] = 1.0;
        z.mm_last_q[0] = 1.0;
        z.mm_ang_vel[0] = 1.0;
        z.optimized.q[0] = z.predicted.q[0] = 1.0;
        z.out_R[0] = z.out_R[4] = z.out_R[8] = 1.0;
        z.out_status = 1;
        z.pnp_seq = (seq_t)c->enq;
        z.early_state = 4u * (seq_t)c->enq + 3u;
        z.track_done_seq = (seq_t)c->enq;
        z.late_gate_seq = (seq_t)c->enq;
        z.gate_timeouts = c->gate_timeouts_seen, z.gate_fatal = c->gate_fatal_seen;
        HIPCHK(c, hipMemcpyAsync(c->d_ctl[s], &z, sizeof(Ctl), hipMemcpyHostToDevice, c->stream));
        HIPCHK(c, hipMemsetAsync(c->h_seqs[s].map_n, 0, sizeof(int), c->stream));
        HIPCHK(c, hipMemsetAsync(c->h_seqs[s].map_cur, 0, sizeof(int), c->stream));
        HIPCHK(c, hipMemsetAsync(c->h_seqs[s].staged_n, 0, sizeof(int), c->stream));
        HIPCHK(c, hipMemsetAsync(c->h_seqs[s].staged_cur, 0, sizeof(int), c->stream));
        for (int r = 0; r < RING; r++) c->h_ctl[r * c->B + s] = z;
    }
    HIPCHK(c, hipStreamSynchronize(c->stream));
}

static bool build_mixed_tables(const std::vector<Params> &ps, std::vector<uint32_t> &cells, std::vector<uint32_t> &score) {
    struct Ent {
        int area;
        uint32_t v;
    };
    std::vector<Ent> es;
    cells.clear(), score.clear();
    for (size_t s = 0; s < ps.size(); s++) {
        const Params &p = ps[s];
        const int eyes = (p.sensor == 2) ? 1 : 2;
        for (int cc = 0; cc < p.n_cells; cc++) {
            const int cx = cc % p.cells_x, cy = cc / p.cells_x;
            const int area = std::min(p.cell_size, p.W - cx * p.cell_size) * std::min(p.cell_size, p.H - cy * p.cell_size);
            for (int e = 0; e < eyes; e++) es.push_back({area, (uint32_t)s << 16 | (uint32_t)e << 8 | (uint32_t)cc});
        }
        const int tx = (p.W + TS_W - 1) / TS_W, ty = (p.H + TS_H - 1) / TS_H;
        if (tx > MIXED_TILE_COLS || ty > MIXED_TILE_ROWS) return false;
        for (int e = 0; e < eyes; e++) {
            const size_t off = score.size(), n = (size_t)tx * ty;
            const uint32_t img = (uint32_t)(2 * s + e);
            score.resize(off + n);
            uint32_t t = 0;
            for (size_t x = 0; x < 8; x++)
                for (size_t g = off + ((x - off) & 7); g < off + n; g += 8, t++) score[g] = img << 22 | (t / (uint32_t)tx) << 8 | (t % (uint32_t)tx);
        }
    }
    std::stable_sort(es.begin(), es.end(), [](const Ent &a, const Ent &b) { return a.area > b.area; });
    for (const Ent &e : es) cells.push_back(e.v);
    return true;
}

static Context *create_context(const lvt_amd_params *in, bool mixed, int sensor, int B, int device) {
    if (sensor != 1 && sensor != 2) return nullptr;
    std::vector<Params> prms(mixed ? B : 1);
    for (size_t s = 0; s < prms.size(); s++)
        if (!derive_params(in[s], sensor, prms[s])) return nullptr;
    const Params prm = prms[0];
    std::vector<uint32_t> cells_tab, score_tab;
    if (mixed && !build_mixed_tables(prms, cells_tab, score_tab)) return nullptr;
    int ndev = 0;
    if (hipGetDeviceCount(&ndev) != hipSuccess || ndev <= 0) return nullptr;
    int cur = 0;
    if (hipGetDevice(&cur) != hipSuccess) return nullptr;
    if (device < 0) device = cur;
    if (device >= ndev) return nullptr;
    Context *c = new Context();
    c->device = device;
    DeviceGuard guard(c);
    try {
        c->count_in(device);
        c->B = B;
        c->sensor = sensor;
        c->prm = prm;
        c->mixed = mixed;
        if (mixed) c->prms = prms;
        c->in_prms.assign(in, in + prms.size());
        for (const Params &q : prms) {
            c->any_staged = c->any_staged || q.staged_th > 0;
            c->any_strips = c->any_strips || q.big_cell_strips != 0;
            c->max_cells = std::max(c->max_cells, q.n_cells);
        }
        HIPCHK(c, hipStreamCreateWithFlags(&c->stream, hipStreamNonBlocking));
        {
            int ncu = 0;
            if (B >= 2 && B <= 28) {
                int total = 0;
                if (hipDeviceGetAttribute(&total, hipDeviceAttributeMultiprocessorCount, device) == hipSuccess && total >= 64) ncu = total / 8 * 7;
            }
            if (const char *e = std::getenv("LVT_AMD_FEATURE_CUS")) ncu = (B >= 2) ? std::atoi(e) : 0;
            if (ncu > 0 && ncu < 1024) {
                uint32_t mask[32] = {};
                for (int i = 0; i < ncu; i++) mask[i >> 5] |= 1u << (i & 31);
                HIPCHK(c, hipExtStreamCreateWithCUMask(&c->stream_f, 32, mask));
                c->feature_cus = ncu;
            } else
                HIPCHK(c, hipStreamCreateWithFlags(&c->stream_f, hipStreamNonBlocking));
        }
        HIPCHK(c, hipStreamCreateWithFlags(&c->stream_e, hipStreamNonBlocking));
        c->own_stream = true;
        for (auto &e : c->ev_done) HIPCHK(c, hipEventCreateWithFlags(&e, hipEventDisableTiming));
        for (auto &e : c->ev_feat) HIPCHK(c, hipEventCreateWithFlags(&e, hipEventDisableTiming));
        HIPCHK(c, hipEventCreateWithFlags(&c->ev_depth, hipEventDisableTiming));
        HIPCHK(c, hipEventCreateWithFlags(&c->ev_switch, hipEventDisableTiming));
        HIPCHK(c, hipEventCreateWithFlags(&c->ev_switch_e, hipEventDisableTiming));
        if (const char *e = std::getenv("LVT_AMD_TEST_GATE_TIMEOUT")) c->test_gate_timeout = std::atol(e);
        {
            const char *o = std::getenv("LVT_AMD_ORDERING");
            if (o && std::strcmp(o, "events") == 0) c->events_only = true;
            else if (o && std::strcmp(o, "polling") == 0) c->events_only = false, c->ordering_forced = true;
            else c->events_only = B == 1 && c->live_on_device() > 1;
        }
        c->pitch = ((prm.W + 63) / 64) * 64;
        HIPCHK(c, hipHostMalloc((void **)&c->h_ctl, sizeof(Ctl) * B * RING, hipHostMallocCoherent));
        HIPCHK(c, hipHostGetDevicePointer((void **)&c->h_ctl_dev, c->h_ctl, 0));
        HIPCHK(c, hipHostMalloc((void **)&c->h_done, sizeof(seq_t) * B * RING, hipHostMallocCoherent));
        HIPCHK(c, hipHostGetDevicePointer((void **)&c->h_done_dev, c->h_done, 0));
        std::memset(c->h_done, 0, sizeof(seq_t) * B * RING);
        HIPCHK(c, hipHostMalloc((void **)&c->h_pose, sizeof(PoseRec) * B * RING, hipHostMallocCoherent));
        HIPCHK(c, hipHostGetDevicePointer((void **)&c->h_pose_dev, c->h_pose, 0));
        HIPCHK(c, hipHostMalloc((void **)&c->h_pose_done, sizeof(seq_t) * B * RING, hipHostMallocCoherent));
        HIPCHK(c, hipHostGetDevicePointer((void **)&c->h_pose_done_dev, c->h_pose_done, 0));
        std::memset(c->h_pose_done, 0, sizeof(seq_t) * B * RING);
        if (const char *e = std::getenv("LVT_AMD_SYNC_TAIL")) c->early_pose = std::strcmp(e, "wait") != 0;
        c->binned_lists = B > 1;
        if (const char *e = std::getenv("LVT_AMD_BINNED_LISTS")) c->binned_lists = std::atoi(e) != 0;
        if (const char *e = std::getenv("LVT_AMD_TEST_ROW_FALLBACK")) c->force_row_fallback = std::atoi(e) != 0;
        {
            int idx[CELLS_MAX], area[CELLS_MAX];
            for (int cc = 0; cc < prm.n_cells; cc++) {
                const int cx = cc % prm.cells_x, cy = cc / prm.cells_x;
                idx[cc] = cc;
                area[cc] = std::min(prm.cell_size, prm.W - cx * prm.cell_size) * std::min(prm.cell_size, prm.H - cy * prm.cell_size);
            }
            std::stable_sort(idx, idx + prm.n_cells, [&](int a, int b) { return area[a] > area[b]; });
            for (int cc = 0; cc < CELLS_MAX; cc++) c->cell_order.v[cc] = (uint8_t)(cc < prm.n_cells ? idx[cc] : 0);
        }
        if (const char *e = std::getenv("LVT_AMD_BRIEF_FROM_IMAGE")) c->brief_from_image = std::atoi(e) ? 1 : 0;
        if (const char *e = std::getenv("LVT_AMD_SCORE_PIECES")) c->score_pieces = std::max(1, std::min(8, std::atoi(e))), c->score_pieces_auto = false;
        {
            int n_cu = 256;
            (void)hipDeviceGetAttribute(&n_cu, hipDeviceAttributeMultiprocessorCount, c->device);
            if (!mixed && !prm.big_cell_strips && prm.n_cells * 2 * B > n_cu) c->cells_raw_cap = RAW_CAP_SMALL;
            if (mixed && !c->any_strips && (int)cells_tab.size() > n_cu) c->cells_raw_cap = RAW_CAP_SMALL;
        }
        if (mixed) c->score_pieces = 1, c->score_pieces_auto = false;
        if (const char *e = std::getenv("LVT_AMD_CELL_SPLIT")) c->cell_split = std::max(0, std::min(SPLIT_MAX, std::atoi(e)));
        if (const char *e = std::getenv("LVT_AMD_CELLS_RAW_CAP")) c->cells_raw_cap = std::max(RAW_CAP_SMALL, std::min(RAW_CAP, std::atoi(e) & ~1));
        if (const char *e = std::getenv("LVT_AMD_FUSED_PULL")) c->fuse_pull = std::atoi(e) != 0;
        c->lists_wgs_row = c->lists_wgs_map = (B <= 16) ? 4 : 2;
        if (const char *e = std::getenv("LVT_AMD_LISTS_WGS")) {
            int r = 0, m = 0;
            const int got = std::sscanf(e, "%d,%d", &r, &m);
            if (got >= 1) c->lists_wgs_row = std::max(1, std::min(64, r));
            if (got >= 2) c->lists_wgs_map = std::max(1, std::min(64, m));
        }
        if (const char *e = std::getenv("LVT_AMD_MATCH_BLOCKS_BATCH")) c->match_blocks_batch = std::max(1, std::min(256, std::atoi(e)));
        HIPCHK(c, hipHostMalloc((void **)&c->h_fargs, sizeof(FrameArgs) * B * RING, hipHostMallocDefault));
        std::memset(c->h_fargs, 0, sizeof(FrameArgs) * B * RING);
        c->h_seqs.resize(B);
        c->d_ctl.resize(B);
        for (int s = 0; s < B; s++) {
            const Params &q = prms[mixed ? s : 0];
            const int pitch = ((q.W + 63) / 64) * 64;
            const size_t plane = (size_t)pitch * q.H;
            Seq &S = c->h_seqs[s];
            std::memset(&S, 0, sizeof(S));
            S.prm = q;
            S.ctl = c->d_ctl[s] = c->dalloc<Ctl>(1);
            S.plane_pitch = pitch;
            {
                size_t off = 0;
                for (int cc = 0; cc < q.n_cells; cc++) {
                    const int cx = cc % q.cells_x, cy = cc / q.cells_x;
                    const int cw = std::min(q.cell_size, q.W - cx * q.cell_size), ch = std::min(q.cell_size, q.H - cy * q.cell_size);
                    S.cell_scratch_off[cc] = off;
                    off += (size_t)cw * ch * 6;
                }
            }
            for (int e = 0; e < 2; e++) S.cell_scratch[e] = c->dalloc<uint32_t>((size_t)q.W * q.H * 6 + 64);
            for (int e = 0; e < 2; e++) {
                S.strip_kp[e] = q.big_cell_strips ? c->dalloc<uint32_t>((size_t)q.n_cells * STRIPS * RAW_CAP) : c->dalloc_uncached<uint32_t>((size_t)q.n_cells * SPLIT_MAX * SPLIT_KP_CAP);
                S.strip_n[e] = c->dalloc_uncached<int>((size_t)CELLS_MAX * STRIPS);
                S.cell_big[e] = c->dalloc<int>(CELLS_MAX);
            }
            S.lists_fb = c->dalloc<int>(2);
            for (int par = 0; par < NPAR; par++) {
                FrameBuf &FB = S.fb[par];
                FB.fc = c->dalloc<FeatCtl>(1);
                for (int e = 0; e < 2; e++) {
                    FB.score[e] = c->dalloc<uint8_t>(plane + 64);
                    FB.boxsum[e] = c->dalloc<uint16_t>(plane + 64);
                    {
                        const size_t tiles_x = (size_t)(q.W + TS_W - 1) / TS_W;
                        FB.seg_keys[e] = c->dalloc<uint32_t>((size_t)q.H * tiles_x * TS_W);
                        FB.seg_cnt[e] = c->dalloc<uint16_t>((size_t)q.H * tiles_x);
                    }
                    FB.cell_kp[e] = c->dalloc<float>((size_t)CELLS_MAX * CELL_OUT_CAP * 3);
                    FB.cell_n[e] = c->dalloc<int>(CELLS_MAX);
                    alloc_feat(c, FB.feat[e]);
                    if (s == 0) {
                        c->d_ext[par][e] = c->dalloc<float>((size_t)EXT_MAX * 2);
                        c->d_img[par][e] = c->dalloc<uint8_t>(plane + 64);
                    }
                    FB.ext_xy[e] = FB.ext_xy_own[e] = c->d_ext[par][e];
                }
                if (s == 0 && sensor == 2) c->d_depth[par] = c->dalloc<float>((size_t)q.W * q.H + 4);
            }
            for (int k = 0; k < 2; k++) {
                alloc_points(c, S.map[k], MAP_MAX);
                alloc_points(c, S.staged[k], STAGED_MAX);
            }
            S.map_cur = c->dalloc<int>(1), S.map_n = c->dalloc<int>(1);
            S.staged_cur = c->dalloc<int>(1), S.staged_n = c->dalloc<int>(1);
            S.proj = c->dalloc<float>((size_t)MAP_MAX * 2);
            S.vis = c->dalloc<int8_t>(MAP_MAX);
            S.match = c->dalloc<int>(MAP_MAX);
            S.cand = c->dalloc<uint32_t>((size_t)MAP_MAX * KC);
            S.ncand = c->dalloc<int>(MAP_MAX);
            S.qidx = c->dalloc<uint32_t>(MAP_MAX);
            S.sproj = c->dalloc<float>((size_t)STAGED_MAX * 2);
            S.svis = c->dalloc<int8_t>(STAGED_MAX);
            S.smatch = c->dalloc<int>(STAGED_MAX);
            S.scand = c->dalloc<uint32_t>((size_t)STAGED_MAX * KC);
            S.sncand = c->dalloc<int>(STAGED_MAX);
            S.sdel = c->dalloc<uint8_t>(STAGED_MAX);
            S.pnp_X = c->dalloc<double>((size_t)NF_MAX * 3);
            S.pnp_obs = c->dalloc<float>((size_t)NF_MAX * 2);
            S.pnp_feat = c->dalloc<int>(NF_MAX);
            S.pnp_err = c->dalloc<double>((size_t)NF_MAX * 2 + 2);
            S.pnp_level = c->dalloc<int8_t>(NF_MAX);
            S.rcand = c->dalloc<uint32_t>((size_t)NPAR * NF_MAX * KC);
            S.rncand = c->dalloc<int>(NPAR * NF_MAX);
            S.pair_l = c->dalloc<int>(NF_MAX), S.pair_r = c->dalloc<int>(NF_MAX);
            S.tri_X = c->dalloc<double>((size_t)NF_MAX * 3);
            S.tri_ok = c->dalloc<int8_t>(NF_MAX);
        }
        c->d_seqs = c->dalloc<Seq>(B);
        HIPCHK(c, hipMemcpy(c->d_seqs, c->h_seqs.data(), sizeof(Seq) * B, hipMemcpyHostToDevice));
        if (mixed) {
            c->n_score_wgs = (int)score_tab.size(), c->n_cells_wgs = (int)cells_tab.size();
            c->d_score_tab = c->dalloc<uint32_t>(score_tab.size());
            c->d_cells_tab = c->dalloc<uint32_t>(cells_tab.size());
            HIPCHK(c, hipMemcpy(c->d_score_tab, score_tab.data(), sizeof(uint32_t) * score_tab.size(), hipMemcpyHostToDevice));
            HIPCHK(c, hipMemcpy(c->d_cells_tab, cells_tab.data(), sizeof(uint32_t) * cells_tab.size(), hipMemcpyHostToDevice));
            HIPCHK(c, hipFuncSetAttribute(reinterpret_cast<const void *>(&k_cells_mixed), hipFuncAttributeMaxDynamicSharedMemorySize, CELLS_LDS_BYTES));
        }
        HIPCHK(c, hipFuncSetAttribute(reinterpret_cast<const void *>(&k_cells<true>), hipFuncAttributeMaxDynamicSharedMemorySize, CELLS_LDS_BYTES));
        HIPCHK(c, hipFuncSetAttribute(reinterpret_cast<const void *>(&k_cells<false>), hipFuncAttributeMaxDynamicSharedMemorySize, CELLS_LDS_BYTES));
        HIPCHK(c, hipFuncSetAttribute(reinterpret_cast<const void *>(&k_hamming_batched_lists<MODE_MAP, true>), hipFuncAttributeMaxDynamicSharedMemorySize, LS_LDS_BYTES));
        HIPCHK(c, hipFuncSetAttribute(reinterpret_cast<const void *>(&k_hamming_batched_lists<MODE_MAP, false>), hipFuncAttributeMaxDynamicSharedMemorySize, LS_LDS_BYTES));
        HIPCHK(c, hipFuncSetAttribute(reinterpret_cast<const void *>(&k_hamming_batched_lists<MODE_ROW, true>), hipFuncAttributeMaxDynamicSharedMemorySize, LS_LDS_BYTES));
        HIPCHK(c, hipFuncSetAttribute(reinterpret_cast<const void *>(&k_hamming_batched_lists<MODE_ROW, false>), hipFuncAttributeMaxDynamicSharedMemorySize, LS_LDS_BYTES));
        HIPCHK(c, hipFuncSetAttribute(reinterpret_cast<const void *>(&k_cells_strip), hipFuncAttributeMaxDynamicSharedMemorySize, CELLS_LDS_BYTES));
        HIPCHK(c, hipFuncSetAttribute(reinterpret_cast<const void *>(&k_gather<true>), hipFuncAttributeMaxDynamicSharedMemorySize, CELLS_LDS_BYTES));
        HIPCHK(c, hipFuncSetAttribute(reinterpret_cast<const void *>(&k_gather<false>), hipFuncAttributeMaxDynamicSharedMemorySize, CELLS_LDS_BYTES));
        HIPCHK(c, hipFuncSetAttribute(reinterpret_cast<const void *>(&k_cells_big), hipFuncAttributeMaxDynamicSharedMemorySize, CELLS_LDS_BYTES));
        HIPCHK(c, hipFuncSetAttribute(reinterpret_cast<const void *>(&k_cells_radii), hipFuncAttributeMaxDynamicSharedMemorySize, CELLS_LDS_BYTES));
        HIPCHK(c, hipFuncSetAttribute(reinterpret_cast<const void *>(&k_cells_select), hipFuncAttributeMaxDynamicSharedMemorySize, CELLS_LDS_BYTES));
        HIPCHK(c, hipFuncSetAttribute(reinterpret_cast<const void *>(&k_pnp<true>), hipFuncAttributeMaxDynamicSharedMemorySize, PNP_DYN_BYTES));
        HIPCHK(c, hipFuncSetAttribute(reinterpret_cast<const void *>(&k_pnp<false>), hipFuncAttributeMaxDynamicSharedMemorySize, PNP_DYN_BYTES));
        reset_state(c);
    } catch (...) {
        delete c;
        return nullptr;
    }
    return c;
}
static Context *create_context(const lvt_amd_params &in, int sensor, int B, int device = -1) { return create_context(&in, false, sensor, B, device); }

static const char *kProfNames[Context::PROF_SLOTS] = {
    "k_feat_begin", "k_gate [early stream: waits for the previous k_pnp]", "k_score", "k_cells(pass0)", "", "k_gather(+ the rare retry pass)", "k_brief", "k_gate_late [waits for the early stream]",
    "k_match_map(wait for the early stream + begin + new points)", "k_early_map [early stream]", "k_early_mid [early stream]", "k_hamming_batched_lists(map) [early stream]", "k_track_mid(resolve+pass2+bookkeep+cull)", "k_pnp(+project staged)", "",
    "", "k_candidates(staged)", "", "k_candidates(row) [early stream]", "k_hamming_batched_lists(row)", "k_triangulate(staged update+row resolve+triangulate+finalize)", "",
    "", ""};

#define LAUNCH(slot, st, kern, grid, block, lds, ...)                              \
    do {                                                                           \
        if (c->prof) (void)hipEventRecord(c->ev[slot][0], st);                     \
        hipLaunchKernelGGL(kern, grid, block, lds, st, __VA_ARGS__);               \
        if (c->prof) {                                                             \
            (void)hipEventRecord(c->ev[slot][1], st);                              \
            c->ev_used[slot] = true;                                               \
        }                                                                          \
    } while (0)

#define LAUNCH_S(slot, st, kern, grid, block, lds, ...)                                                      \
    do {                                                                                                     \
        if (B == 1) LAUNCH(slot, st, kern<true>, grid, block, lds, SeqArg<true>{c->h_seqs[0]}, __VA_ARGS__); \
        else LAUNCH(slot, st, kern<false>, grid, block, lds, SeqArg<false>{S}, __VA_ARGS__);                  \
    } while (0)
#define LAUNCH_SM(slot, st, kern, MODE_, grid, block, lds, ...)                                                        \
    do {                                                                                                               \
        if (B == 1) LAUNCH(slot, st, (kern<MODE_, true>), grid, block, lds, SeqArg<true>{c->h_seqs[0]}, __VA_ARGS__);   \
        else LAUNCH(slot, st, (kern<MODE_, false>), grid, block, lds, SeqArg<false>{S}, __VA_ARGS__);                   \
    } while (0)

static void collect_oldest(Context *c);

struct HostTimer {
    double *acc;
    std::chrono::steady_clock::time_point t0;
    explicit HostTimer(double *a) : acc(a), t0(std::chrono::steady_clock::now()) {}
    ~HostTimer() { *acc += std::chrono::duration<double, std::micro>(std::chrono::steady_clock::now() - t0).count(); }
};
static void enqueue_frame(Context *c) {
    HostTimer ht(&c->host_enq_us);
    c->host_enq_n++;
    const int B = c->B;
    const int Bz = (c->launch_seqs > 0 && c->launch_seqs < B) ? c->launch_seqs : B;
    c->ring_seqs[(int)(c->enq % RING)] = Bz;
    const Params &p = c->prm;
    Seq *S = c->d_seqs;
    const int slot = (int)(c->enq % RING), par = (int)(c->enq % NPAR);
    if (c->want_events && !c->events_only) {
        if (c->enq > 0 && c->delivered < c->enq) {
            const int pslot = (int)((c->enq - 1) % RING);
            hipLaunchKernelGGL(k_deliver, dim3(1, 1, Bz), dim3(64), 0, c->stream, S, c->h_ctl_dev + (size_t)pslot * B, c->h_done_dev + (size_t)pslot * B, (seq_t)c->enq);
            c->delivered = c->enq;
        }
        (void)hipEventRecord(c->ev_switch_e, c->stream_e);
        (void)hipStreamWaitEvent(c->stream, c->ev_switch_e, 0);
        (void)hipStreamWaitEvent(c->stream_f, c->ev_switch_e, 0);
        (void)hipEventRecord(c->ev_switch, c->stream);
        (void)hipStreamWaitEvent(c->stream_f, c->ev_switch, 0);
        c->events_only = true;
        c->want_events = false;
        c->switched_at = (long)c->enq;
    }
    const FrameArgs *fa = c->h_fargs + (size_t)slot * B;
    const int ext = (B == 1) ? fa[0].ext_corners : 0;
    hipStream_t sf = c->stream_f, st = c->stream;
    for (int i = 0; i < Context::PROF_SLOTS; i++) c->ev_used[i] = false;
    const bool evo = c->events_only;
    const bool feat_pack = B > 1 && Bz <= FEAT_PACK && !std::getenv("LVT_AMD_NO_FEAT_PACK");
    if (c->enq >= NPAR) {
        if (!evo && !feat_pack)
            hipLaunchKernelGGL(k_gate_buf, dim3(1, 1, Bz), dim3(64), 0, sf, S, (seq_t)(c->enq + 1 - NPAR), par);
        else if (c->switched_at < 0 || (long)c->enq - NPAR >= c->switched_at)
            (void)hipStreamWaitEvent(sf, c->ev_done[(int)((c->enq - NPAR) % RING)], 0);
    }
    if (B == 1) {
        LAUNCH(2, sf, k_score<true>, dim3((p.W + TS_W - 1) / TS_W, (p.H + TS_H - 1) / TS_H, 2), dim3(256), 0, S, c->h_fargs[slot], par, 0, c->brief_from_image ? 0 : 1);
    } else {
        if (feat_pack) {
            FrameArgsPack pk;
            std::memset(&pk, 0, sizeof(pk));
            for (int s = 0; s < Bz; s++) pk.a[s] = fa[s];
            LAUNCH(0, sf, k_feat_begin_pack, dim3(Bz), dim3(64), 0, S, pk, par, (seq_t)((c->enq >= NPAR && !evo) ? c->enq + 1 - NPAR : 0));
        } else
            LAUNCH(0, sf, k_feat_begin, dim3(Bz), dim3(64), 0, S, fa, par);
        if (c->mixed) {
            LAUNCH(2, sf, k_score_mixed, dim3(c->n_score_wgs), dim3(256), 0, S, c->d_score_tab, par, c->brief_from_image ? 0 : 1);
        } else {
            const int P = std::max(1, std::min(c->score_pieces, Bz));
            for (int q = 0; q < P; q++) {
                const int z0 = 2 * (int)((long)Bz * q / P), z1 = 2 * (int)((long)Bz * (q + 1) / P);
                if (q == 0) LAUNCH(2, sf, k_score<false>, dim3((p.W + TS_W - 1) / TS_W, (p.H + TS_H - 1) / TS_H, z1 - z0), dim3(256), 0, S, FrameArgs{}, par, z0, c->brief_from_image ? 0 : 1);
                else hipLaunchKernelGGL(k_score<false>, dim3((p.W + TS_W - 1) / TS_W, (p.H + TS_H - 1) / TS_H, z1 - z0), dim3(256), 0, sf, S, FrameArgs{}, par, z0, c->brief_from_image ? 0 : 1);
            }
        }
    }
    if (!ext) {
        {
            const int pass = 0;
            const int pull_wgs = (B == 1 && c->next_pull.src[0]) ? std::min(64, (int)(((size_t)p.W * p.H / 16 + 1023) / 1024)) : 0;
            const int ns = (B == 1 && !p.big_cell_strips) ? c->cell_split : 0;
            const int gx = (ns >= 2) ? ((((p.n_cells + 7) & ~7) * ns + pull_wgs + 7) & ~7) : p.n_cells + pull_wgs;
            if (c->mixed) LAUNCH(3, sf, k_cells_mixed, dim3(c->n_cells_wgs), dim3(1024), cells_lds_bytes(c->cells_raw_cap), (const Seq *)S, c->d_cells_tab, pass, par, c->cells_raw_cap);
            else LAUNCH_S(3, sf, k_cells, (B == 1 ? dim3(gx, 2, 1) : dim3(p.n_cells * 2 * Bz, 1, 1)), dim3(1024), cells_lds_bytes(c->cells_raw_cap), pass, par, c->cell_order, 2 * Bz, c->cells_raw_cap, c->next_pull, ns, (++c->cell_token ? c->cell_token : ++c->cell_token));
            if (c->any_strips) {
                const int nc = c->max_cells;
                hipLaunchKernelGGL(k_cells_strip, dim3(nc * STRIPS, 2, Bz), dim3(1024), CELLS_LDS_BYTES, sf, S, pass, par);
                hipLaunchKernelGGL(k_cells_big, dim3(nc, 2, Bz), dim3(1024), CELLS_LDS_BYTES, sf, S, pass, par);
                hipLaunchKernelGGL(k_cells_radii, dim3(nc * RADII_WGS, 2, Bz), dim3(1024), CELLS_LDS_BYTES, sf, S, pass, par);
                hipLaunchKernelGGL(k_cells_select, dim3(nc, 2, Bz), dim3(1024), CELLS_LDS_BYTES, sf, S, pass, par);
                if (c->prof) (void)hipEventRecord(c->ev[3][1], sf);
            }
        }
    }
    if (c->before_gather) {
        c->before_gather();
        c->before_gather = nullptr;
    }
    if (c->depth_wait) {
        (void)hipStreamWaitEvent(sf, c->ev_depth, 0);
        c->depth_wait = false;
    }
    LAUNCH_S(5, sf, k_gather, dim3(1, 2, Bz), dim3(1024), CELLS_LDS_BYTES, (const Seq *)S, par);
    const bool brief_publishes = !evo && B == 1;
    if (c->brief_from_image) LAUNCH_S(6, sf, k_brief_img, dim3(64, 2, Bz), dim3(256), 0, (const Seq *)S, par, brief_publishes ? (seq_t)(c->enq + 1) : (seq_t)0);
    else LAUNCH_S(6, sf, k_brief, dim3(64, 2, Bz), dim3(256), 0, (const Seq *)S, par, brief_publishes ? (seq_t)(c->enq + 1) : (seq_t)0);
    if (!evo && !brief_publishes) hipLaunchKernelGGL(k_feat_done, dim3(Bz), dim3(64), 0, sf, S, par, (seq_t)(c->enq + 1));
    const int bl = c->binned_lists ? 1 : 0;
    if (evo && bl && c->sensor == 1) LAUNCH_SM(19, sf, k_hamming_batched_lists, MODE_ROW, dim3(c->lists_wgs_row, 1, Bz), dim3(LS_THREADS), LS_LDS_BYTES, par, (seq_t)0);
    if (evo) LAUNCH_SM(18, sf, k_candidates, MODE_ROW, dim3(256, 1, Bz), dim3(256), 0, 0, par, (seq_t)0, bl);
    if (evo) hipLaunchKernelGGL(k_feat_done, dim3(Bz), dim3(64), 0, sf, S, par, (seq_t)(c->enq + 1));
    if (evo) (void)hipEventRecord(c->ev_feat[par], sf);
    const seq_t seq = (seq_t)(c->enq + 1);
    if (!evo) {
        hipStream_t se = c->stream_e;
        LAUNCH_S(1, se, k_gate, dim3(1, 1, Bz), dim3(64), 0, par, (seq_t)c->enq, seq, (c->test_gate_timeout && (long)seq == c->test_gate_timeout) ? 1 : 0);
        if (bl) LAUNCH_SM(11, se, k_hamming_batched_lists, MODE_MAP, dim3(c->lists_wgs_map, 1, Bz), dim3(LS_THREADS), LS_LDS_BYTES, par, seq);
        LAUNCH_S(9, se, k_early_map, dim3((bl && B > 1) ? 32 : 256, 1, Bz), dim3(256), 0, par, seq, bl);
        LAUNCH_S(10, se, k_early_mid, dim3(1, 1, Bz), dim3(RES_THREADS), 0, par, seq);
        if (c->sensor == 1) {
            if (bl) LAUNCH_SM(19, se, k_hamming_batched_lists, MODE_ROW, dim3(c->lists_wgs_row, 1, Bz), dim3(LS_THREADS), LS_LDS_BYTES, par, seq);
            LAUNCH_SM(18, se, k_candidates, MODE_ROW, dim3(B == 1 ? ROW_BLOCKS : ROW_BLOCKS_BATCH, 1, Bz), dim3(256), 0, 0, par, seq, bl);
            hipLaunchKernelGGL(k_row_done, dim3(Bz), dim3(64), 0, se, S, par, seq);
        }
    }
    {
        Ctl *prec = nullptr;
        seq_t *pdone = nullptr;
        if (!evo && c->delivered < c->enq) {
            const int pslot = (int)((c->enq - 1) % RING);
            prec = c->h_ctl_dev + (size_t)pslot * B, pdone = c->h_done_dev + (size_t)pslot * B;
            c->delivered = c->enq;
        }
        if (evo) {
            (void)hipStreamWaitEvent(st, c->ev_feat[par], 0);
            LAUNCH_S(8, st, k_match_map, dim3(256, 1, Bz), dim3(256), 0, par, seq, 0, (Ctl *)nullptr, (seq_t *)nullptr);
        } else if (B == 1 && c->live_on_device() <= MAX_FOLDED_GATES) {
            LAUNCH_S(8, st, k_match_map, dim3(MATCH_BLOCKS_GATED, 1, 1), dim3(256), 0, par, seq, 1, prec, pdone);
        } else {
            LAUNCH_S(7, st, k_gate_late, dim3(1, 1, Bz), dim3(64), 0, par, seq, prec, pdone);
            LAUNCH_S(8, st, k_match_map, dim3(B > 1 ? c->match_blocks_batch : 256, 1, Bz), dim3(256), 0, par, seq, 0, (Ctl *)nullptr, (seq_t *)nullptr);
        }
    }
    LAUNCH_S(12, st, k_track_mid, dim3(1, 1, Bz), dim3(RES_THREADS), 0, par, seq);
    {
        const bool ep = c->sync_call && c->early_pose && !c->prof && B == 1;
        LAUNCH_S(13, st, k_pnp, dim3(1, 1, Bz), dim3(PNP_THREADS), PNP_DYN_BYTES, par, seq, ep ? c->h_pose_dev + (size_t)slot * B : (PoseRec *)nullptr,
                 ep ? c->h_pose_done_dev + (size_t)slot * B : (seq_t *)nullptr);
    }
    if (c->any_staged)
        LAUNCH_SM(16, st, k_candidates, MODE_STAGED, dim3(64, 1, Bz), dim3(256), 0, 0, par, (seq_t)0, 0);
    LAUNCH_S(20, st, k_triangulate, dim3(1, 1, Bz), dim3(1024), 0, par, seq, c->h_ctl_dev + (size_t)slot * B,
           c->h_done_dev + (size_t)slot * B, evo ? 0 : (c->force_row_fallback ? 2 : 1), (evo || c->sync_call) ? 1 : 0);
    if (evo || c->sync_call) c->delivered = c->enq + 1;
    if (evo) (void)hipEventRecord(c->ev_done[slot], st);
    c->enq++;
}

static void collect_oldest(Context *c) {
    HostTimer ht(&c->host_wait_us);
    c->host_wait_n++;
    if (c->done >= c->enq) return;
    const int slot = (int)(c->done % RING);
    const int Bz = (c->ring_seqs[slot] > 0 && c->ring_seqs[slot] <= c->B) ? c->ring_seqs[slot] : c->B;
    if (c->delivered < c->done + 1) {
        hipLaunchKernelGGL(k_deliver, dim3(1, 1, Bz), dim3(64), 0, c->stream, c->d_seqs, c->h_ctl_dev + (size_t)slot * c->B,
                           c->h_done_dev + (size_t)slot * c->B, (seq_t)(c->done + 1));
        c->delivered = c->done + 1;
    }
    {
        const seq_t want = (seq_t)(c->done + 1);
        unsigned spins = 0;
        for (int s = 0; s < Bz; s++) {
            volatile seq_t *f = c->h_done + (size_t)slot * c->B + s;
            while (__atomic_load_n(f, __ATOMIC_ACQUIRE) != want) {
                __builtin_ia32_pause();
                if ((++spins & 0xFFFFF) == 0) {
                    const hipError_t q = hipStreamQuery(c->stream);
                    if (q != hipSuccess && q != hipErrorNotReady) {
                        c->set_error(std::string("tracking stream: ") + hipGetErrorString(q));
                        s = c->B;
                        break;
                    }
                    if (q == hipSuccess && __atomic_load_n(f, __ATOMIC_ACQUIRE) != want) {
                        c->set_error("tracking stream finished without a result record");
                        s = c->B;
                        break;
                    }
                }
            }
        }
        if (c->prof) HIPCHK(c, hipStreamSynchronize(c->stream));
    }
    c->last_slot = slot;
    c->last_par = (int)(c->done % NPAR);
    c->done++;
    hipError_t e = hipGetLastError();
    if (e != hipSuccess) c->set_error(std::string("kernel chain: ") + hipGetErrorString(e));
    if (c->prof && c->done == c->enq) {
// ... 306 lines not shown
    try {
        DeviceGuard guard(static_cast<Context *>(h));
        delete static_cast<Context *>(h);
    } catch (...) {
    }
}

LVT_API void lvt_amd_reset(lvt_handle h) {
    h = resolve_handle(h);
    if (is_slot(h)) {
        try {
            View v;
            if (view_of(h, v)) reset_state(v.c, v.s);
            PoolSlot *S = static_cast<PoolSlot *>(h);
            std::memset(&S->last.rec, 0, sizeof(Ctl));
            S->last.rec.state = S->last.rec.out_status = 1;
            S->last.rec.out_R[0] = S->last.rec.out_R[4] = S->last.rec.out_R[8] = 1.0;
            S->last.rec.last_pose.q[0] = S->last.rec.predicted.q[0] = 1.0;
        } catch (...) {
        }
        return;
    }
    try {
        DeviceGuard guard(static_cast<Context *>(h));
        reset_state(static_cast<Context *>(h));
    } catch (...) {
    }
}

LVT_API void lvt_amd_set_stream(lvt_handle h, void *hip_stream) {
    h = resolve_handle(h);
    if (!is_ctx(h)) return;
    Context *c = static_cast<Context *>(h);
    DeviceGuard guard(c);
    try {
        drain(c);
        if (c->own_stream && c->stream) (void)hipStreamDestroy(c->stream);
        c->stream = static_cast<hipStream_t>(hip_stream);
        c->own_stream = false;
    } catch (...) {
    }
}

LVT_API const char *lvt_amd_last_error(lvt_handle h) {
    if (is_auto(h)) {
        AutoHandle *A = static_cast<AutoHandle *>(h);
        std::lock_guard<std::mutex> g(A->mu);
        static thread_local std::string acopy;
        acopy = lvt_amd_last_error(A->impl);
        return acopy.c_str();
    }
    if (!h) return "no handle (creation failed: bad parameters, or no HIP device -- there is no CPU fallback)";
    if (is_slot(h)) {
        PoolSlot *S = static_cast<PoolSlot *>(h);
        std::lock_guard<std::mutex> g(S->pool->mu);
        static thread_local std::string copy;
        copy = S->err;
        return copy.c_str();
    }
    Context *c = static_cast<Context *>(h);
    if (c->early_pending) {
        DeviceGuard guard(c);
        try {
            drain(c);
        } catch (...) {
        }
    }
    return c->err.c_str();
}

LVT_API void lvt_amd_get_host_stats(lvt_handle h, long long out[8]) {
    h = resolve_handle(h);
    Context *c = static_cast<Context *>(h);
    for (int i = 0; i < 8; i++) out[i] = 0;
    if (!c) return;
    if (is_slot(h)) {
        PoolSlot *S = static_cast<PoolSlot *>(h);
        std::lock_guard<std::mutex> g(S->pool->mu);
        out[0] = S->submitted, out[1] = S->pool->steps, out[2] = S->pool->slot_frames, out[3] = S->pool->live, out[7] = 2;
        return;
    }
    out[0] = (long long)c->enq + (c->pend.valid ? 1 : 0), out[1] = (long long)c->done, out[2] = c->planes_in_place, out[3] = c->planes_staged;
    out[4] = c->async_frames, out[5] = c->fused_pulls, out[6] = c->score_pieces, out[7] = c->events_only ? 1 : 0;
}

LVT_API void lvt_amd_profile_enable(lvt_handle h, int enable) {
    h = resolve_handle(h);
    if (!is_ctx(h)) return;
    Context *c = static_cast<Context *>(h);
    DeviceGuard guard(c);
    try {
        drain(c);
        if (enable) {
            for (auto &e : c->ev)
                for (auto &x : e)
                    if (!x) HIPCHK(c, hipEventCreate(&x));
            for (int i = 0; i < Context::PROF_SLOTS; i++) c->prof_ms[i] = 0, c->prof_calls[i] = 0;
        }
        c->prof = enable != 0;
    } catch (...) {
    }
}
LVT_API int lvt_amd_profile_read(lvt_handle h, int slot, char *name, int name_cap, double *total_ms, long *calls) {
    h = resolve_handle(h);
    if (!is_ctx(h)) return 0;
    Context *c = static_cast<Context *>(h);
    DeviceGuard guard(c);
    if (slot < 0 || slot >= Context::PROF_SLOTS || !kProfNames[slot][0]) return 0;
    std::snprintf(name, name_cap, "%s", kProfNames[slot]);
    *total_ms = c->prof_ms[slot];
    *calls = c->prof_calls[slot];
    return 1;
}

LVT_API void lvt_amd_track_device_async(lvt_handle h, const void *d_left, const void *d_right, int n_rows, int n_cols, int pitch_bytes) {
    h = resolve_handle(h);
    if (is_slot(h)) {
        try {
            (void)slot_submit(static_cast<PoolSlot *>(h), static_cast<const uint8_t *>(d_left), static_cast<const uint8_t *>(d_right), n_rows, n_cols, pitch_bytes, false);
        } catch (...) {
        }
        return;
    }
    Context *c = static_cast<Context *>(h);
    DeviceGuard guard(c);
    try {
        if (c->sensor != 1) {
            c->set_error("lvt_amd_track_device: a stereo entry point on an RGB-D handle (the frame was NOT enqueued; use lvt_amd_track_rgbd_device)");
            return;
        }
        if (!size_ok(c, n_rows, n_cols) || (pitch_bytes & 15)) {
            c->set_error("lvt_amd_track_device: image size / pitch mismatch");
            return;
        }
        if (c->early_pending) drain(c);
        make_room(c);
        FrameArgs &f = c->h_fargs[(size_t)(c->enq % RING) * c->B];
        f.img[0] = static_cast<const uint8_t *>(d_left);
        f.img[1] = static_cast<const uint8_t *>(d_right);
        f.depth = nullptr;
        f.img_pitch = pitch_bytes;
        f.depth_pitch = 0;
        f.depth_format = DEPTH_F32, f.depth_scale = 0.f;
        f.ext_corners = 0;
        f.absent = 0;
        f.n_ext[0] = f.n_ext[1] = 0;
        enqueue_frame(c);
    } catch (...) {
    }
}

LVT_API lvt_handle lvt_amd_batch_create(const lvt_amd_params *p, int sensor_type, int n_sequences) {
    try {
        if (n_sequences < 1 || n_sequences > 256) return nullptr;
        return static_cast<lvt_handle>(create_context(*p, sensor_type, n_sequences));
    } catch (...) {
    }
    return nullptr;
}
LVT_API lvt_handle lvt_amd_batch_create_mixed(const lvt_amd_params *p, int sensor_type, int n_sequences) {
    try {
        if (!p || n_sequences < 1 || n_sequences > 256) return nullptr;
        return static_cast<lvt_handle>(create_context(p, true, sensor_type, n_sequences, -1));
    } catch (...) {
    }
    return nullptr;
// ... 1211 lines not shown
```

Before: 9177.

## Fuse early-stream gate, list build and map resolve into one LDS-resident kernel

Adds a single-workgroup k_early kernel that replaces k_gate on the early stream for single-sequence, non-binned runs. It waits for features, bins train features into LDS by hash cell, builds the candidate lists and resolves map matches in one launch. k_early_map, k_early_mid and the map list kernel then return early when fused_seq matches. The aim is to cut launch count and global-memory round trips on the early-stream critical path. In exchange it adds a mid_seq handshake from k_pnp, a large dynamic LDS footprint, a slow-path fallback and a stand-down path when the map exceeds the thread count.

```diff
diff --git a/include/lvt_amd_ext.h b/include/lvt_amd_ext.h
--- a/include/lvt_amd_ext.h
+++ b/include/lvt_amd_ext.h
@@ -72,6 +72,7 @@
 LVT_API const char *lvt_amd_last_error(lvt_handle h);
 
 LVT_API void lvt_amd_get_host_stats(lvt_handle h, long long out[8]);
+LVT_API void lvt_amd_get_early_stats(lvt_handle h, long long out[2]);
 
 LVT_API void lvt_amd_profile_enable(lvt_handle h, int enable);
 LVT_API int lvt_amd_profile_read(lvt_handle h, int slot, char *name, int name_cap, double *total_ms, long *calls);
diff --git a/lvt_amd/__init__.py b/lvt_amd/__init__.py
--- a/lvt_amd/__init__.py
+++ b/lvt_amd/__init__.py
@@ -21,7 +21,7 @@
     "lvt_amd_rectify_device", "lvt_amd_rectify", "lvt_amd_rectifier_get_maps",
     "lvt_amd_odometry_create", "lvt_amd_odometry_destroy", "lvt_amd_odometry_reset", "lvt_amd_odometry_push_pose", "lvt_amd_odometry_update", "lvt_amd_profile_enable", "lvt_amd_profile_read", "lvt_amd_get_debug", "lvt_amd_get_timeline", "lvt_amd_get_ordering",
     "lvt_amd_batch_create", "lvt_amd_batch_size", "lvt_amd_batch_track_device_async", "lvt_amd_batch_wait",
-    "lvt_amd_batch_get_counts", "lvt_amd_create_on_device", "lvt_amd_get_device", "lvt_amd_wait_status", "lvt_amd_get_host_stats",
+    "lvt_amd_batch_get_counts", "lvt_amd_create_on_device", "lvt_amd_get_device", "lvt_amd_wait_status", "lvt_amd_get_host_stats", "lvt_amd_get_early_stats",
     "lvt_amd_track_async", "lvt_amd_track_rgbd_async", "lvt_amd_pnp_trace", "lvt_amd_create_pooled", "lvt_amd_wait_pose",
     "lvt_amd_batch_create_mixed", "lvt_amd_batch_track_device_async_mixed", "lvt_amd_batch_get_params", "lvt_amd_batch_mixed_tables",
     "lvt_amd_track_rgbd_device", "lvt_amd_track_rgbd_device_async", "lvt_amd_track_rgbd16", "lvt_amd_track_rgbd16_async",
@@ -143,6 +143,7 @@
             fn.argtypes, fn.restype = argtypes, C.c_int
     L.lvt_amd_get_debug.argtypes = [vp, vp]
     L.lvt_amd_get_host_stats.argtypes = [vp, vp]
+    L.lvt_amd_get_early_stats.argtypes = [vp, vp]
     L.lvt_amd_profile_read.argtypes = [vp, C.c_int, C.c_char_p, C.c_int, vp, vp]
     _lib = L
     return L
@@ -217,8 +218,11 @@
     def host_stats(self) -> dict:
         a = (C.c_longlong * 8)()
         load_library().lvt_amd_get_host_stats(self._h, a)
+        e = (C.c_longlong * 2)()
+        load_library().lvt_amd_get_early_stats(self._h, e)
         return {"enqueued": int(a[0]), "collected": int(a[1]), "planes_in_place": int(a[2]), "planes_staged": int(a[3]),
-                "async_host_frames": int(a[4]), "pulls_carried_by_the_previous_frame": int(a[5]), "score_pieces": int(a[6]), "event_ordering": int(a[7])}
+                "async_host_frames": int(a[4]), "pulls_carried_by_the_previous_frame": int(a[5]), "score_pieces": int(a[6]), "event_ordering": int(a[7]),
+                "early_fused_frames": int(e[0]), "early_fused_standdowns": int(e[1])}
 
     def track(self, img1, img2, depth_scale=None):
         R = np.zeros((3, 3)); t = np.zeros(3)
diff --git a/lvt_amd/csrc/k_features.hip b/lvt_amd/csrc/k_features.hip
--- a/lvt_amd/csrc/k_features.hip
+++ b/lvt_amd/csrc/k_features.hip
@@ -866,11 +866,9 @@
                 misc[2] = 0;
             }
             __syncthreads();
-            int levels = 0;
             while (true) {
                 const int cnt = misc[1];
                 if (cnt == 0) break;
-                levels++;
                 if (cnt >= DFS_AT) {
                     for (int sgi = wave_id(); sgi < cnt; sgi += nw)
                         wave_introsort_segment<I>(arr, qa[3 * sgi], qa[3 * sgi + 1], qa[3 * sgi + 2], posL, posR, stacks + 96 * wave_id());
@@ -905,7 +903,6 @@
                 __syncthreads();
             }
             __syncthreads();
-            if (dbg && tid == 0) dbg[41] = levels;
         }
         STAMP(6);
         int *hist = row_first;
diff --git a/lvt_amd/csrc/k_lists.hip b/lvt_amd/csrc/k_lists.hip
--- a/lvt_amd/csrc/k_lists.hip
+++ b/lvt_amd/csrc/k_lists.hip
@@ -29,6 +29,7 @@
     int *fb = S.lists_fb + (MODE == MODE_ROW ? 1 : 0);
     int q_end = 0;
     if (MODE == MODE_MAP) {
+        if (ctl.fused_seq == seq) return;
         const int n_early = (ctl.gate_ok == seq) ? ctl.early_done : 0;
         if (n_early <= 0) return;
         q_end = min(*S.map_n, n_early);
diff --git a/lvt_amd/csrc/k_track.hip b/lvt_amd/csrc/k_track.hip
--- a/lvt_amd/csrc/k_track.hip
+++ b/lvt_amd/csrc/k_track.hip
@@ -451,6 +451,7 @@
     const Seq &S = sa.get();
     if (only_fb && !S.lists_fb[0]) return;
     Ctl &ctl = *S.ctl;
+    if (ctl.fused_seq == seq) return;
     const int n_early = (ctl.gate_ok == seq) ? ctl.early_done : 0;
     if (n_early <= 0) return;
     __shared__ double w2c[12];
@@ -562,7 +563,7 @@
 template <class NFn>
 __device__ __forceinline__ int resolve_super(int b0, int M, NFn nfn, const uint32_t *cand, ResolveLds &L, uint32_t &iter, float ratio,
                                              float desc_th, int acc[2], int nq[2] = nullptr, const uint32_t *qidx = nullptr, int qid[2] = nullptr,
-                                             bool no_marks = false) {
+                                             bool no_marks = false, const uint32_t *pre = nullptr) {
     const int tid = threadIdx.x;
     int n[2], off[2], qq[2];
     const long long ts0 = clock64();
@@ -587,6 +588,12 @@
 #pragma unroll
     for (int u = 0; u < 2; u++)
         if (tid + u * RES_THREADS >= limit) n[u] = 0;
+    long long ts1 = ts0;
+    if (pre) {
+#pragma unroll
+        for (int u = 0; u < 2; u++) off[u] = (n[u] > 0) ? (int)(pre[qq[u]] & 0xFFFFu) : 0;
+        if (nq) nq[0] = n[0], nq[1] = n[1];
+    } else {
     const int n4[2] = {(n[0] + 3) & ~3, (n[1] + 3) & ~3};
     int t0, t1;
     off[0] = block_excl_scan(n4[0], L.scan, &t0);
@@ -606,7 +613,7 @@
         for (int u = 0; u < 2; u++)
             if (tid + u * RES_THREADS >= limit) n[u] = 0;
     }
-    const long long ts1 = clock64();
+    ts1 = clock64();
     if (nq) nq[0] = n[0], nq[1] = n[1];
 #pragma unroll
     for (int u = 0; u < 2; u++) {
@@ -646,6 +653,7 @@
             }
         }
         n[u] = w;
+    }
     }
     if (tid == 0) L.misc[12] = L.misc[13] = QCAP;
     __syncthreads();
@@ -1115,6 +1123,7 @@
     if (threadIdx.x == 0 && blockIdx.x == 0) sa.get().ctl->dbg[36] = (long long)wall_clock64();
     const Seq &S = sa.get();
     Ctl &ctl = *S.ctl;
+    if (ctl.fused_seq == seq) return;
     const int n_early = (ctl.gate_ok == seq) ? ctl.early_done : 0;
     if (n_early > 0) {
         RESOLVE_LDS_DECL
@@ -1126,6 +1135,461 @@
         ctl.dbg[37] = (long long)wall_clock64();
         __threadfence();
         if (n_early > 0 || ctl.gate_ok == seq) atomicCAS(&ctl.early_state, 4u * seq + 1u, 4u * seq + 2u);
+    }
+}
+
+constexpr int EF_THREADS = RES_THREADS;
+constexpr int EF_WAVES = EF_THREADS / 64;
+constexpr int EF_TPT = 2;
+constexpr int EF_NMAX = 1536;
+constexpr int EF_BINS = 1100;
+constexpr int EF_STARTS = (EF_BINS + 2 + 3) & ~3;
+constexpr int EF_SEG = 256;
+constexpr int EF_DYN_BYTES = 160 * 1024 - 768;
+constexpr int EF_FIXED_BYTES = EF_STARTS * 4 + EF_THREADS * 4 + EF_WAVES * EF_SEG * 4;
+static_assert(EF_TPT * EF_THREADS >= EF_NMAX, "every train feature has a thread");
+static_assert(KC + 64 <= EF_SEG, "the long-window path shares the wavefront's segment words");
+static_assert(EF_NMAX * 51 + EF_FIXED_BYTES + 4096 * 4 <= EF_DYN_BYTES, "a list area is left at the feature capacity");
+static_assert(EF_NMAX <= NF_MAX && EF_DYN_BYTES / 4 < 65536, "list starts are 16-bit words");
+typedef unsigned int ef_u32x4 __attribute__((ext_vector_type(4)));
+
+__device__ __forceinline__ uint32_t ef_shfl(uint32_t v, int src) { return (uint32_t)__builtin_amdgcn_ds_bpermute(src << 2, (int)v); }
+__device__ __forceinline__ ef_u32x4 ef_shfl4(ef_u32x4 v, int src) { return ef_u32x4{ef_shfl(v.x, src), ef_shfl(v.y, src), ef_shfl(v.z, src), ef_shfl(v.w, src)}; }
+__device__ __forceinline__ uint32_t ef_ham(ef_u32x4 d0, ef_u32x4 d1, ef_u32x4 a0, ef_u32x4 a1) {
+    return (uint32_t)(__popc(d0.x ^ a0.x) + __popc(d0.y ^ a0.y) + __popc(d0.z ^ a0.z) + __popc(d0.w ^ a0.w) + __popc(d1.x ^ a1.x) + __popc(d1.y ^ a1.y) +
+                      __popc(d1.z ^ a1.z) + __popc(d1.w ^ a1.w));
+}
+__device__ __forceinline__ bool early_claim(Ctl &ctl, seq_t seq, bool ok) {
+    const seq_t mine = 4u * seq + (ok ? 1u : 3u);
+    seq_t cur = __hip_atomic_load(&ctl.early_state, __ATOMIC_ACQUIRE, __HIP_MEMORY_SCOPE_AGENT);
+    for (;;) {
+        if (cur >= 4u * seq + 1u) {
+            ok = false;
+            break;
+        }
+        const seq_t seen = atomicCAS(&ctl.early_state, cur, mine);
+        if (seen == cur) break;
+        cur = seen;
+    }
+    return ok;
+}
+
+__global__ __launch_bounds__(EF_THREADS) void k_early(SeqArg<true> sa, int par, seq_t want, seq_t seq, int test_timeout) {
+    const Seq &S = sa.get();
+    Ctl &ctl = *S.ctl;
+    FeatCtl &fc = *S.fb[par].fc;
+    const int tid = threadIdx.x, lane = tid & 63, wv = tid >> 6;
+    extern __shared__ __attribute__((aligned(16))) uint8_t ef_smem[];
+    __shared__ int s_scan[32];
+    __shared__ int s_misc[16];
+    __shared__ double w2c[12];
+    __shared__ int s_v[8];
+    __shared__ float s_qxy[2];
+
+    if (tid == 0) {
+        ctl.dbg[32] = (long long)wall_clock64();
+        bool ok = true;
+        if (test_timeout) {
+            atomicAdd(&ctl.gate_timeouts, 1);
+            ok = false;
+        } else {
+            const unsigned long long t0 = wall_clock64();
+            while (__hip_atomic_load(&fc.feat_seq, __ATOMIC_ACQUIRE, __HIP_MEMORY_SCOPE_AGENT) < seq) {
+                __builtin_amdgcn_s_sleep(8);
+                if (wall_clock64() - t0 > 2000000ull) {
+                    atomicAdd(&ctl.gate_timeouts, 1);
+                    ok = false;
+                    break;
+                }
+            }
+            if (ok && __hip_atomic_load(&fc.skip_seq, __ATOMIC_ACQUIRE, __HIP_MEMORY_SCOPE_AGENT) == seq) ok = false;
+            ctl.dbg[35] = (long long)wall_clock64();
+        }
+        s_v[0] = ok ? 1 : 0, s_v[1] = 0, s_v[2] = 0, s_v[3] = 0, s_v[4] = 1;
+    }
+    __syncthreads();
+    if (!s_v[0]) {
+        if (tid == 0) {
+            early_claim(ctl, seq, false);
+            ctl.gate_ok = 0;
+            ctl.dbg[33] = (long long)wall_clock64();
+        }
+        return;
+    }
+    __builtin_amdgcn_fence(__ATOMIC_ACQUIRE, "agent");
+
+    const Feat &T = S.fb[par].feat[0];
+    const int N = __hip_atomic_load(T.n, __ATOMIC_RELAXED, __HIP_MEMORY_SCOPE_AGENT);
+    const int ccx = S.prm.hash_ccx, ccy = S.prm.hash_ccy, csr = S.prm.cell_search_radius;
+    const int nbins = ccx * ccy;
+    const bool fit_a = N <= EF_NMAX && nbins <= EF_BINS && csr <= 2;
+    const int Nr = fit_a ? max((N + 15) & ~15, 16) : 16;
+    ef_u32x4 *s_dlo = reinterpret_cast<ef_u32x4 *>(ef_smem);
+    ef_u32x4 *s_dhi = s_dlo + Nr;
+    float2 *s_xy = reinterpret_cast<float2 *>(s_dhi + Nr);
+    uint32_t *s_tab0 = reinterpret_cast<uint32_t *>(s_xy + Nr), *s_tab1 = s_tab0 + Nr;
+    int *s_start = reinterpret_cast<int *>(s_tab1 + Nr);
+    uint32_t *s_qno = reinterpret_cast<uint32_t *>(s_start + EF_STARTS);
+    uint32_t *s_seg = s_qno + EF_THREADS + wv * EF_SEG;
+    uint16_t *s_idx = reinterpret_cast<uint16_t *>(s_qno + EF_THREADS + EF_WAVES * EF_SEG);
+    uint8_t *s_flag = reinterpret_cast<uint8_t *>(s_idx + Nr);
+    uint32_t *s_lists = reinterpret_cast<uint32_t *>(s_flag + Nr);
+    const int lists_cap = ((EF_DYN_BYTES - Nr * 51 - EF_FIXED_BYTES) / 4) & ~3;
+
+    float tx[EF_TPT], ty[EF_TPT];
+    int tbin[EF_TPT], trank[EF_TPT];
+    ef_u32x4 tlo[EF_TPT], thi[EF_TPT];
+    if (fit_a) {
+#pragma unroll
+        for (int k = 0; k < EF_TPT; k++) {
+            const int jc = max(min(tid + k * EF_THREADS, N - 1), 0);
+            tx[k] = ty[k] = 0.f, tbin[k] = nbins, trank[k] = 0;
+            tlo[k] = thi[k] = ef_u32x4{0, 0, 0, 0};
+            if (N > 0) {
+                tx[k] = T.x[jc], ty[k] = T.y[jc];
+                const int cy = T.hcy[jc], cx = T.hcx[jc];
+                tbin[k] = (cy >= 0 && cy < ccy && cx >= 0 && cx < ccx) ? cy * ccx + cx : nbins;
+                const ef_u32x4 *d = reinterpret_cast<const ef_u32x4 *>(T.desc + (size_t)jc * 4);
+                tlo[k] = d[0], thi[k] = d[1];
+            }
+        }
+        for (int i = tid; i < nbins + 2; i += EF_THREADS) s_start[i] = 0;
+        for (int j = tid; j < Nr; j += EF_THREADS) s_tab0[j] = s_tab1[j] = 0u, s_flag[j] = 0;
+        __syncthreads();
+#pragma unroll
+        for (int k = 0; k < EF_TPT; k++)
+            if (tid + k * EF_THREADS < N) trank[k] = atomicAdd(&s_start[tbin[k]], 1);
+        __syncthreads();
+        {
+            const int chunk = (nbins + 2 + EF_THREADS - 1) / EF_THREADS;
+            const int i0 = min(tid * chunk, nbins + 2), i1 = min(i0 + chunk, nbins + 2);
+            int sum = 0;
+            for (int i = i0; i < i1; i++) sum += s_start[i];
+            int total;
+            int run = block_excl_scan(sum, s_scan, &total);
+            for (int i = i0; i < i1; i++) {
+                const int v = s_start[i];
+                s_start[i] = run;
+                run += v;
+            }
+        }
+        __syncthreads();
+#pragma unroll
+        for (int k = 0; k < EF_TPT; k++) {
+            const int j = tid + k * EF_THREADS;
+            if (j < N) {
+                const int pos = s_start[tbin[k]] + trank[k];
+                s_xy[pos] = make_float2(tx[k], ty[k]);
+                s_idx[pos] = (uint16_t)j;
+                s_dlo[pos] = tlo[k];
+                s_dhi[pos] = thi[k];
+            }
+        }
+    }
+
+    if (tid == 0 && fit_a) {
+        const unsigned long long t0 = wall_clock64();
+        while (__hip_atomic_load(&ctl.mid_seq, __ATOMIC_ACQUIRE, __HIP_MEMORY_SCOPE_AGENT) < want) {
+            __builtin_amdgcn_s_sleep(8);
+            if (wall_clock64() - t0 > 2000000ull) {
+                s_v[4] = 0;
+                break;
+            }
+        }
+    }
+    __syncthreads();
+    __builtin_amdgcn_fence(__ATOMIC_ACQUIRE, "agent");
+    const int cur = __hip_atomic_load(S.map_cur, __ATOMIC_RELAXED, __HIP_MEMORY_SCOPE_AGENT);
+    const int n_st = (fit_a && s_v[4]) ? min(__hip_atomic_load(S.map_n, __ATOMIC_RELAXED, __HIP_MEMORY_SCOPE_AGENT), EF_THREADS) : 0;
+    const MapSoA &P = S.map[cur];
+    double X[3] = {0, 0, 0};
+    ef_u32x4 qd0 = {0, 0, 0, 0}, qd1 = {0, 0, 0, 0};
+    int pcounter = 0;
+    if (tid < n_st) {
+        X[0] = P.pos[3 * tid], X[1] = P.pos[3 * tid + 1], X[2] = P.pos[3 * tid + 2];
+        const ef_u32x4 *d = reinterpret_cast<const ef_u32x4 *>(P.desc + (size_t)tid * 4);
+        qd0 = d[0], qd1 = d[1];
+        pcounter = P.counter[tid];
+    }
+
+    if (tid == 0) {
+        bool ok = true;
+        const unsigned long long t1 = wall_clock64();
+        ctl.dbg[41] = (long long)t1;
+        while (__hip_atomic_load(&ctl.pnp_seq, __ATOMIC_ACQUIRE, __HIP_MEMORY_SCOPE_AGENT) < want) {
+            __builtin_amdgcn_s_sleep(1);
+            if (wall_clock64() - t1 > 2000000ull) {
+                atomicAdd(&ctl.gate_timeouts, 1);
+                ok = false;
+                break;
+            }
+        }
+        ok = early_claim(ctl, seq, ok);
+        ctl.gate_ok = ok ? seq : (seq_t)0;
+        const long long tg = (long long)wall_clock64();
+        ctl.dbg[33] = tg, ctl.dbg[34] = tg;
+        int n_early = 0;
+        if (ok) {
+            n_early = ctl.early_done;
+            if (n_early > 0 && n_early <= n_st) {
+                Pose predicted;
+                double mmn[14];
+                motion_predict(ctl, ctl.last_pose, predicted, mmn);
+                world_to_camera(predicted, w2c);
+            }
+        }
+        s_v[0] = ok ? 1 : 0, s_v[1] = n_early;
+    }
+    __syncthreads();
+    if (!s_v[0]) return;
+    const int n_early = s_v[1];
+    if (n_early <= 0) {
+        if (tid == 0) {
+            ctl.fused_seq = seq;
+            ctl.fused_frames += 1;
+            ctl.dbg[37] = (long long)wall_clock64();
+            __threadfence();
+            atomicCAS(&ctl.early_state, 4u * seq + 1u, 4u * seq + 2u);
+        }
+        return;
+    }
+    if (n_early > n_st) {
+        if (tid == 0) ctl.fused_standdowns += 1;
+        return;
+    }
+
+    const int radius = S.prm.tracking_radius;
+    const float r2 = (float)(radius * radius);
+    bool live = false;
+    double u = 0, v = 0;
+    ef_u32x4 W0 = {0, 0, 0, 0}, W1 = {0, 0, 0, 0};
+    if (tid < n_early) {
+        live = is_point_visible(X, w2c, S.prm, u, v);
+        if (live) {
+            Query Q;
+            make_query_track(S.prm, (float)u, (float)v, radius, Q);
+            uint32_t rg[5] = {0, 0, 0, 0, 0};
+            int total = 0;
+            if (Q.sx < Q.ex) {
+#pragma unroll
+                for (int k = 0; k < 5; k++) {
+                    const int r = Q.sy + k;
+                    if (r < Q.ey) {
+                        const int s0 = s_start[r * ccx + Q.sx], l0 = s_start[r * ccx + Q.ex] - s0;
+                        rg[k] = (uint32_t)s0 | ((uint32_t)l0 << 16), total += l0;
+                    }
+                }
+            }
+            W0 = ef_u32x4{(uint32_t)total, __float_as_uint(Q.x), __float_as_uint(Q.y), rg[0]};
+            W1 = ef_u32x4{rg[1], rg[2], rg[3], rg[4]};
+        }
+    }
+    s_qno[tid] = 0u;
+    __builtin_amdgcn_wave_barrier();
+
+    {
+        const int row = lane >> 4, sl = lane & 15;
+        const uint32_t my_total = W0.x;
+        auto long_window = [&](int src) {
+            const ef_u32x4 V0 = ef_shfl4(W0, src), V1 = ef_shfl4(W1, src), d0 = ef_shfl4(qd0, src), d1 = ef_shfl4(qd1, src);
+            const int total = __builtin_amdgcn_readfirstlane((int)V0.x);
+            const float qx = __uint_as_float(V0.y), qy = __uint_as_float(V0.z);
+            const int l0 = (int)(V0.w >> 16), l1 = (int)(V1.x >> 16), l2 = (int)(V1.y >> 16), l3 = (int)(V1.z >> 16);
+            const int c1 = l0, c2 = c1 + l1, c3 = c2 + l2, c4 = c3 + l3;
+            const int o0 = (int)(V0.w & 0xFFFFu), o1 = (int)(V1.x & 0xFFFFu) - c1, o2 = (int)(V1.y & 0xFFFFu) - c2, o3 = (int)(V1.z & 0xFFFFu) - c3,
+                      o4 = (int)(V1.w & 0xFFFFu) - c4;
+            int n = 0;
+            for (int vb = 0; vb < total; vb += 64) {
+                const int vv = vb + lane;
+                const bool in = vv < total;
+                int pos = vv + o0;
+                pos = (vv >= c1) ? vv + o1 : pos;
+                pos = (vv >= c2) ? vv + o2 : pos;
+                pos = (vv >= c3) ? vv + o3 : pos;
+                pos = (vv >= c4) ? vv + o4 : pos;
+                pos = in ? pos : 0;
+                const float2 c = s_xy[pos];
+                const uint32_t id = s_idx[pos];
+                const ef_u32x4 a0 = s_dlo[pos], a1 = s_dhi[pos];
+                const float dx = c.x - qx, dy = c.y - qy;
+                const bool ok = ((dx * dx + dy * dy) < r2) && in;
+                const uint32_t d = ef_ham(d0, d1, a0, a1);
+                const uint64_t bal = __ballot(ok);
+                const int slot = n + (int)__builtin_amdgcn_mbcnt_hi((uint32_t)(bal >> 32), __builtin_amdgcn_mbcnt_lo((uint32_t)bal, 0u));
+                if (ok && slot < KC + 64) s_seg[slot] = (d << 16) | id;
+                n += __popcll(bal);
+            }
+            if (n > KC) {
+                if (lane == 0) s_qno[wv * 64 + src] = (uint32_t)min(n, 0xFFFF) << 16;
+            } else if (n > 0) {
+                const int n4 = (n + 3) & ~3;
+                if (lane < n4 - n) s_seg[n + lane] = 0xFFFFFFFFu;
+                __builtin_amdgcn_wave_barrier();
+                uint32_t off = 0;
+                if (lane == 0) off = (uint32_t)atomicAdd(&s_v[2], n4);
+                off = (uint32_t)__builtin_amdgcn_readfirstlane((int)off);
+                if ((int)off + n4 > lists_cap) {
+                    if (lane == 0) s_v[3] = 1;
+                } else {
+                    const uint4 *seg4 = reinterpret_cast<const uint4 *>(s_seg);
+                    const uint32_t ka = lane < n ? s_seg[lane] : 0xFFFFFFFFu, kb = lane + 64 < n ? s_seg[lane + 64] : 0xFFFFFFFFu;
+                    int ra = 0, rb = 0;
+                    for (int o = 0; o < n; o += 4) {
+                        const uint4 kv = seg4[o >> 2];
+                        ra += (kv.x < ka) + (kv.y < ka) + (kv.z < ka) + (kv.w < ka);
+                        rb += (kv.x < kb) + (kv.y < kb) + (kv.z < kb) + (kv.w < kb);
+                    }
+                    uint32_t *dst = s_lists + off;
+                    if (lane < n) dst[ra] = ka;
+                    if (lane + 64 < n) dst[rb] = kb;
+                    if (lane < n4 - n) dst[n + lane] = 0u;
+                    if (lane == 0) s_qno[wv * 64 + src] = off | ((uint32_t)n << 16);
+                }
+            }
+            __builtin_amdgcn_wave_barrier();
+        };
+        for (int s = 0; s < 16; s++) {
+            const int src = 4 * s + row;
+            const int total = (int)ef_shfl(my_total, src);
+            const int tmax = max(max(__builtin_amdgcn_readlane(total, 0), __builtin_amdgcn_readlane(total, 16)),
+                                 max(__builtin_amdgcn_readlane(total, 32), __builtin_amdgcn_readlane(total, 48)));
+            if (tmax == 0) continue;
+            if (tmax > 64) {
+                for (int r = 0; r < 4; r++)
+                    if (__builtin_amdgcn_readlane(total, 16 * r) > 0) long_window(4 * s + r);
+                continue;
+            }
+            const ef_u32x4 V0 = ef_shfl4(W0, src), V1 = ef_shfl4(W1, src), d0 = ef_shfl4(qd0, src), d1 = ef_shfl4(qd1, src);
+            const float qx = __uint_as_float(V0.y), qy = __uint_as_float(V0.z);
+            const int l0 = (int)(V0.w >> 16), l1 = (int)(V1.x >> 16), l2 = (int)(V1.y >> 16), l3 = (int)(V1.z >> 16);
+            const int c1 = l0, c2 = c1 + l1, c3 = c2 + l2, c4 = c3 + l3;
+            const int o0 = (int)(V0.w & 0xFFFFu), o1 = (int)(V1.x & 0xFFFFu) - c1, o2 = (int)(V1.y & 0xFFFFu) - c2, o3 = (int)(V1.z & 0xFFFFu) - c3,
+                      o4 = (int)(V1.w & 0xFFFFu) - c4;
+            uint32_t *seg = s_seg + row * 64;
+            const int PASSES = (tmax + 15) >> 4;
+            uint32_t K[4] = {0xFFFFFFFFu, 0xFFFFFFFFu, 0xFFFFFFFFu, 0xFFFFFFFFu};
+            int n = 0;
+#pragma unroll
+            for (int p = 0; p < 4; p++) {
+                if (p < PASSES) {
+                    const int vv = p * 16 + sl;
+                    const bool in = vv < total;
+                    int pos = vv + o0;
+                    pos = (vv >= c1) ? vv + o1 : pos;
+                    pos = (vv >= c2) ? vv + o2 : pos;
+                    pos = (vv >= c3) ? vv + o3 : pos;
+                    pos = (vv >= c4) ? vv + o4 : pos;
+                    pos = in ? pos : 0;
+                    const float2 c = s_xy[pos];
+                    const uint32_t id = s_idx[pos];
+                    const ef_u32x4 a0 = s_dlo[pos], a1 = s_dhi[pos];
+                    const float dx = c.x - qx, dy = c.y - qy;
+                    const bool ok = ((dx * dx + dy * dy) < r2) && in;
+                    const uint32_t key = (ef_ham(d0, d1, a0, a1) << 16) | id;
+                    const uint32_t brow = (uint32_t)(__ballot(ok) >> (row * 16)) & 0xFFFFu;
+                    if (ok) {
+                        K[p] = key;
+                        seg[n + __popc(brow & ((1u << sl) - 1u))] = key;
+                    }
+                    n += __popc(brow);
+                }
+            }
+            const int n4 = (n + 3) & ~3;
+            if (sl < n4 - n) seg[n + sl] = 0xFFFFFFFFu;
+            __builtin_amdgcn_wave_barrier();
+            uint32_t off = 0;
+            if (sl == 0 && n > 0) off = (uint32_t)atomicAdd(&s_v[2], n4);
+            off = ef_shfl(off, row * 16);
+            const bool room = (int)off + n4 <= lists_cap;
+            if (sl == 0 && n > 0 && !room) s_v[3] = 1;
+            const int nmax = max(max(__builtin_amdgcn_readlane(n, 0), __builtin_amdgcn_readlane(n, 16)), max(__builtin_amdgcn_readlane(n, 32), __builtin_amdgcn_readlane(n, 48)));
+            const uint4 *seg4 = reinterpret_cast<const uint4 *>(seg);
+            int rk[4] = {0, 0, 0, 0};
+            for (int o = 0; o < nmax; o += 4) {
+                uint4 kv = seg4[o >> 2];
+                if (o >= n) kv = make_uint4(0xFFFFFFFFu, 0xFFFFFFFFu, 0xFFFFFFFFu, 0xFFFFFFFFu);
+#pragma unroll
+                for (int p = 0; p < 4; p++)
+                    if (p < PASSES) rk[p] += (kv.x < K[p]) + (kv.y < K[p]) + (kv.z < K[p]) + (kv.w < K[p]);
+            }
+            if (n > 0 && room) {
+                uint32_t *dst = s_lists + off;
+#pragma unroll
+                for (int p = 0; p < 4; p++)
+                    if (p < PASSES && K[p] != 0xFFFFFFFFu) dst[rk[p]] = K[p];
+                if (sl < n4 - n) dst[n + sl] = 0u;
+                if (sl == 0) s_qno[wv * 64 + src] = off | ((uint32_t)n << 16);
+            }
+            __builtin_amdgcn_wave_barrier();
+        }
+    }
+    __syncthreads();
+    if (s_v[3]) {
+        if (tid == 0) ctl.fused_standdowns += 1;
+        return;
+    }
+
+    if (tid < n_early) {
+        if (live) {
+            S.proj[2 * tid] = (float)u;
+            S.proj[2 * tid + 1] = (float)v;
+            S.vis[tid] = 1;
+            S.match[tid] = -1;
+        } else {
+            S.vis[tid] = 0;
+            P.counter[tid] = pcounter + 1;
+            S.match[tid] = -2;
+        }
+    }
+    if (tid == 0) ctl.dbg[36] = (long long)wall_clock64();
+
+    ResolveLds L;
+    L.flag = s_flag, L.tab0 = s_tab0, L.tab1 = s_tab1, L.lists = s_lists, L.scan = s_scan, L.misc = s_misc;
+    const float ratio = S.prm.track_ratio, desc_th = S.prm.desc_th;
+    uint32_t iter = 0;
+    int accepted = 0;
+    for (int b0 = 0; b0 < n_early;) {
+        int acc[2], nq[2] = {0, 0}, qid[2];
+        const int used = resolve_super(b0, n_early, [&](int q) { return (int)(s_qno[q] >> 16); }, nullptr, L, iter, ratio, desc_th, acc, nq, nullptr, qid, false, s_qno);
+        if (used < 0) {
+            if (tid == b0) s_qxy[0] = (float)u, s_qxy[1] = (float)v;
+            __syncthreads();
+            if (wv == 0) {
+                const int idx = decide_query_slow<MODE_MAP>(S, T, N, L.flag, P.desc, b0, s_qxy[0], s_qxy[1], radius, ratio, desc_th);
+                if (lane == 0) {
+                    S.match[b0] = idx;
+                    if (idx >= 0) {
+                        L.flag[idx] = 1;
+                        L.tab0[idx] = L.tab1[idx] = PERM;
+                    }
+                    L.misc[1] = (idx >= 0) ? 1 : 0;
+                }
+            }
+            __syncthreads();
+            accepted += L.misc[1];
+            __syncthreads();
+            b0 += 1;
+            continue;
+        }
+        const int a0 = (tid < used && acc[0] >= 0) ? 1 : 0;
+        const int tot = __syncthreads_count(a0);
+        if (tid < used && nq[0] > 0) S.match[qid[0]] = acc[0];
+        accepted += tot;
+        b0 += used;
+        __syncthreads();
+    }
+    __syncthreads();
+    for (int j = tid; j < N; j += EF_THREADS) T.flag[j] = L.flag[j];
+    __builtin_amdgcn_fence(__ATOMIC_RELEASE, "agent");
+    __syncthreads();
+    if (tid == 0) {
+        ctl.early_accepted = accepted;
+        ctl.early_ran_seq = seq;
+        ctl.fused_seq = seq;
+        ctl.fused_frames += 1;
+        ctl.dbg[37] = (long long)wall_clock64();
+        __threadfence();
+        atomicCAS(&ctl.early_state, 4u * seq + 1u, 4u * seq + 2u);
     }
 }
 
@@ -1642,6 +2106,7 @@
     if (threadIdx.x == 0 && blockIdx.x == 0) sa.get().ctl->dbg[44] = (long long)wall_clock64();
     const Seq &S = sa.get();
     Ctl &ctl = *S.ctl;
+    if (threadIdx.x == PNP_THREADS - 1) __hip_atomic_store(&ctl.mid_seq, seq, __ATOMIC_RELEASE, __HIP_MEMORY_SCOPE_AGENT);
     if (!ctl.active || ctl.first_frame || ctl.lost_now) {
         if (threadIdx.x == 0) {
             __threadfence();
diff --git a/lvt_amd/csrc/lvt_dev.h b/lvt_amd/csrc/lvt_dev.h
--- a/lvt_amd/csrc/lvt_dev.h
+++ b/lvt_amd/csrc/lvt_dev.h
@@ -71,6 +71,8 @@
     seq_t early_state;
     seq_t track_done_seq;
     seq_t late_gate_seq;
+    seq_t mid_seq, fused_seq;
+    int fused_frames, fused_standdowns;
     int gate_timeouts;
     int gate_fatal;
     int skip;
diff --git a/lvt_amd/csrc/lvt_host.hip b/lvt_amd/csrc/lvt_host.hip
--- a/lvt_amd/csrc/lvt_host.hip
+++ b/lvt_amd/csrc/lvt_host.hip
@@ -123,6 +123,8 @@
     PoseRec *h_pose = nullptr, *h_pose_dev = nullptr;
     seq_t *h_pose_done = nullptr, *h_pose_done_dev = nullptr;
     bool binned_lists = false;
+    bool early_fused = true;
+    bool no_feat_pack = false;
     bool early_pose = true;
     bool early_pending = false;
     FrameArgs *h_fargs = nullptr;
@@ -394,6 +396,7 @@
         z.early_state = 4u * (seq_t)c->enq + 3u;
         z.track_done_seq = (seq_t)c->enq;
         z.late_gate_seq = (seq_t)c->enq;
+        z.mid_seq = (seq_t)c->enq;
         z.gate_timeouts = c->gate_timeouts_seen, z.gate_fatal = c->gate_fatal_seen;
         HIPCHK(c, hipMemcpyAsync(c->d_ctl[s], &z, sizeof(Ctl), hipMemcpyHostToDevice, c->stream));
         HIPCHK(c, hipMemsetAsync(c->h_seqs[s].map_n, 0, sizeof(int), c->stream));
@@ -510,6 +513,8 @@
         if (const char *e = std::getenv("LVT_AMD_SYNC_TAIL")) c->early_pose = std::strcmp(e, "wait") != 0;
         c->binned_lists = B > 1;
         if (const char *e = std::getenv("LVT_AMD_BINNED_LISTS")) c->binned_lists = std::atoi(e) != 0;
+        if (const char *e = std::getenv("LVT_AMD_EARLY_FUSED")) c->early_fused = std::atoi(e) != 0;
+        c->no_feat_pack = std::getenv("LVT_AMD_NO_FEAT_PACK") != nullptr;
         if (const char *e = std::getenv("LVT_AMD_TEST_ROW_FALLBACK")) c->force_row_fallback = std::atoi(e) != 0;
         {
             int idx[CELLS_MAX], area[CELLS_MAX];
@@ -637,6 +642,7 @@
         HIPCHK(c, hipFuncSetAttribute(reinterpret_cast<const void *>(&k_hamming_batched_lists<MODE_MAP, false>), hipFuncAttributeMaxDynamicSharedMemorySize, LS_LDS_BYTES));
         HIPCHK(c, hipFuncSetAttribute(reinterpret_cast<const void *>(&k_hamming_batched_lists<MODE_ROW, true>), hipFuncAttributeMaxDynamicSharedMemorySize, LS_LDS_BYTES));
         HIPCHK(c, hipFuncSetAttribute(reinterpret_cast<const void *>(&k_hamming_batched_lists<MODE_ROW, false>), hipFuncAttributeMaxDynamicSharedMemorySize, LS_LDS_BYTES));
+        HIPCHK(c, hipFuncSetAttribute(reinterpret_cast<const void *>(&k_early), hipFuncAttributeMaxDynamicSharedMemorySize, EF_DYN_BYTES));
         HIPCHK(c, hipFuncSetAttribute(reinterpret_cast<const void *>(&k_cells_strip), hipFuncAttributeMaxDynamicSharedMemorySize, CELLS_LDS_BYTES));
         HIPCHK(c, hipFuncSetAttribute(reinterpret_cast<const void *>(&k_gather<true>), hipFuncAttributeMaxDynamicSharedMemorySize, CELLS_LDS_BYTES));
         HIPCHK(c, hipFuncSetAttribute(reinterpret_cast<const void *>(&k_gather<false>), hipFuncAttributeMaxDynamicSharedMemorySize, CELLS_LDS_BYTES));
@@ -656,7 +662,7 @@
 
 static const char *kProfNames[Context::PROF_SLOTS] = {
     "k_feat_begin", "k_gate [early stream: waits for the previous k_pnp]", "k_score", "k_cells(pass0)", "", "k_gather(+ the rare retry pass)", "k_brief", "k_gate_late [waits for the early stream]",
-    "k_match_map(wait for the early stream + begin + new points)", "k_early_map [early stream]", "k_early_mid [early stream]", "k_hamming_batched_lists(map) [early stream]", "k_track_mid(resolve+pass2+bookkeep+cull)", "k_pnp(+project staged)", "",
+    "k_match_map(wait for the early stream + begin + new points)", "k_early_map [early stream]", "k_early_mid [early stream]", "k_hamming_batched_lists(map) [early stream]", "k_track_mid(resolve+pass2+bookkeep+cull)", "k_pnp(+project staged)", "k_early(gate+lists+resolve; incl. its waits) [early stream]",
     "", "k_candidates(staged)", "", "k_candidates(row) [early stream]", "k_hamming_batched_lists(row)", "k_triangulate(staged update+row resolve+triangulate+finalize)", "",
     "", ""};
 
@@ -718,11 +724,11 @@
     hipStream_t sf = c->stream_f, st = c->stream;
     for (int i = 0; i < Context::PROF_SLOTS; i++) c->ev_used[i] = false;
     const bool evo = c->events_only;
-    const bool feat_pack = B > 1 && Bz <= FEAT_PACK && !std::getenv("LVT_AMD_NO_FEAT_PACK");
+    const bool feat_pack = B > 1 && Bz <= FEAT_PACK && !c->no_feat_pack;
     if (c->enq >= NPAR) {
-        if (!evo && !feat_pack)
-            hipLaunchKernelGGL(k_gate_buf, dim3(1, 1, Bz), dim3(64), 0, sf, S, (seq_t)(c->enq + 1 - NPAR), par);
-        else if (c->switched_at < 0 || (long)c->enq - NPAR >= c->switched_at)
+        if (!evo) {
+            if (!feat_pack) hipLaunchKernelGGL(k_gate_buf, dim3(1, 1, Bz), dim3(64), 0, sf, S, (seq_t)(c->enq + 1 - NPAR), par);
+        } else if (c->switched_at < 0 || (long)c->enq - NPAR >= c->switched_at)
             (void)hipStreamWaitEvent(sf, c->ev_done[(int)((c->enq - NPAR) % RING)], 0);
     }
     if (B == 1) {
@@ -785,7 +791,9 @@
     const seq_t seq = (seq_t)(c->enq + 1);
     if (!evo) {
         hipStream_t se = c->stream_e;
-        LAUNCH_S(1, se, k_gate, dim3(1, 1, Bz), dim3(64), 0, par, (seq_t)c->enq, seq, (c->test_gate_timeout && (long)seq == c->test_gate_timeout) ? 1 : 0);
+        const int gate_test = (c->test_gate_timeout && (long)seq == c->test_gate_timeout) ? 1 : 0;
+        if (B == 1 && c->early_fused && !bl) LAUNCH(14, se, k_early, dim3(1), dim3(EF_THREADS), EF_DYN_BYTES, SeqArg<true>{c->h_seqs[0]}, par, (seq_t)c->enq, seq, gate_test);
+        else LAUNCH_S(1, se, k_gate, dim3(1, 1, Bz), dim3(64), 0, par, (seq_t)c->enq, seq, gate_test);
         if (bl) LAUNCH_SM(11, se, k_hamming_batched_lists, MODE_MAP, dim3(c->lists_wgs_map, 1, Bz), dim3(LS_THREADS), LS_LDS_BYTES, par, seq);
         LAUNCH_S(9, se, k_early_map, dim3((bl && B > 1) ? 32 : 256, 1, Bz), dim3(256), 0, par, seq, bl);
         LAUNCH_S(10, se, k_early_mid, dim3(1, 1, Bz), dim3(RES_THREADS), 0, par, seq);
@@ -1258,6 +1266,15 @@
     }
     out[0] = (long long)c->enq + (c->pend.valid ? 1 : 0), out[1] = (long long)c->done, out[2] = c->planes_in_place, out[3] = c->planes_staged;
     out[4] = c->async_frames, out[5] = c->fused_pulls, out[6] = c->score_pieces, out[7] = c->events_only ? 1 : 0;
+}
+
+LVT_API void lvt_amd_get_early_stats(lvt_handle h, long long out[2]) {
+    out[0] = out[1] = 0;
+    h = resolve_handle(h);
+    if (!is_ctx(h)) return;
+    Context *c = static_cast<Context *>(h);
+    if (c->B != 1) return;
+    out[0] = last_ctl(c).fused_frames, out[1] = last_ctl(c).fused_standdowns;
 }
 
 LVT_API void lvt_amd_profile_enable(lvt_handle h, int enable) {
```

Measured after the change: 7220. -21.3%, worse.
